# vituslcx/Shuffle-exchange

Measured on AMD Instinct MI355X. Metric: tokens/sec Llama-3-8B ZeRO-3 bf16 (training, whole job), higher is better.
Workload: dtype bf16; 1 GPU; llama8b-z3; model=llama3-8b, global_batch=16, seq_len=2048, micro_batch_per_gpu=8, grad_accum=2, parallelism=zero3-dp1, params=8030261248, activation_checkpointing=False, optimizer=AdamW(fp32 master, fused HIP), zero_knobs=tuned, sequence_parallel_size=1, expert_parallel_size=1

## Files before the change

csrc/kernels/flash_attn.hip:

```cpp
#include "sxe_common.h"
#include "sxe_mfma.h"
#include <torch/library.h>
#include <type_traits>

namespace sxe {
namespace fa {
using namespace mf;

constexpr int NW = 4;
constexpr int QW = 32;
constexpr int QB = NW * QW;
constexpr int KT = 64;

template <int D>
struct LaneOffs {
  int row[D / 16];
  int tr[D / 32][2];
  __device__ __forceinline__ void init(int lane) {
    const int r = lane & 31, h = lane >> 5;
#pragma unroll
    for (int t2 = 0; t2 < D / 16; ++t2) row[t2] = soff<D>(r, 2 * t2 + h);
    const int g = lane >> 4, i = lane & 15, q = i >> 2, p = i & 3, hh = g >> 1;
#pragma unroll
    for (int dt = 0; dt < D / 32; ++dt) {
      const int ch = 4 * dt + 2 * (g & 1) + (p >> 1);
      tr[dt][0] = soff<D>(4 * hh + q, ch) + 8 * (p & 1);
      tr[dt][1] = soff<D>(4 * hh + q + 8, ch) + 8 * (p & 1);
    }
  }
};
__device__ __forceinline__ bf16x8 lds_row_at(const char* base, int off) {
  return *reinterpret_cast<const bf16x8*>(base + off);
}
__device__ __forceinline__ bf16x8 lds_tr_at(const char* base, const int (&o)[2]) {
  return tr_pair(lds_tr(base, o[0]), lds_tr(base, o[1]));
}

struct Strides {
  int64_t b, s, h;
};

template <int ROWS, int NWAVES, int D>
struct Stager {
  static constexpr int CH = D / 8;
  static constexpr int N = ROWS * CH / (NWAVES * 64);
  u32x4 r[N];
  __device__ __forceinline__ void load(const unsigned short* base, int64_t row_stride, int row0, int nrows_valid) {
#pragma unroll
    for (int i = 0; i < N; ++i) {
      const int c = threadIdx.x + i * NWAVES * 64;
      const int row = c / CH, ch = c % CH;
      if (row0 + row < nrows_valid)
        r[i] = *reinterpret_cast<const u32x4*>(base + (int64_t)(row0 + row) * row_stride + ch * 8);
      else
        r[i] = u32x4{0, 0, 0, 0};
    }
  }
  __device__ __forceinline__ void store(char* lds) {
#pragma unroll
    for (int i = 0; i < N; ++i) {
      const int c = threadIdx.x + i * NWAVES * 64;
      const int row = c / CH, ch = c % CH;
      const int f = (((row & 3) << 2) | ((row >> 2) & 3)) & (CH >= 16 ? 15 : CH - 1);
      *reinterpret_cast<u32x4*>(lds + (row * (2 * D) + 16 * (ch ^ f))) = r[i];
    }
  }
};

struct Sparse {
  const uint8_t* layout;
  int blk, nb;
};

__device__ __forceinline__ int build_tile_list(const Sparse sp, int head, int t_lo, int t_hi, int tile, int r_lo,
                                               int r_hi, bool fixed_is_query, int* list) {
  int* flags = list + 1024;
  for (int t = t_lo + (int)threadIdx.x; t < t_hi; t += blockDim.x) {
    const int a0 = r_lo / sp.blk, a1 = (r_hi - 1) / sp.blk;
    const int b0 = (t * tile) / sp.blk, b1 = (t * tile + tile - 1) / sp.blk;
    int act = 0;
    for (int a = a0; a <= a1 && !act; ++a)
      for (int bb = b0; bb <= b1; ++bb) {
        const int qb_ = fixed_is_query ? a : bb, kb_ = fixed_is_query ? bb : a;
        if (sp.layout[((int64_t)head * sp.nb + qb_) * sp.nb + kb_]) { act = 1; break; }
      }
    flags[t - t_lo] = act;
  }
  __syncthreads();
  if (threadIdx.x == 0) {
    int n = 0;
    for (int t = t_lo; t < t_hi; ++t)
      if (flags[t - t_lo]) list[n++] = t;
    list[-1] = n;
  }
  __syncthreads();
  return list[-1];
}

struct Band {
  const int* klo;
  const int* qhi;
};
__device__ __forceinline__ int band_klo(const Band& bd, int b, int S, int i) {
  return min(max(bd.klo[(int64_t)b * S + i], 0), i);
}
__device__ __forceinline__ int band_qhi(const Band& bd, int b, int S, int j) {
  return max(min(bd.qhi[(int64_t)b * S + j], S - 1), j);
}

struct Varlen {
  const int* table;
  int T, window;
};

__device__ __forceinline__ void map_block(int nblk, int BH, bool heavy_last_index, int& bh, int& blk) {
  const int idx = blockIdx.x;
  const int rank = idx / BH;
  bh = idx - rank * BH;
  blk = heavy_last_index ? (nblk - 1 - rank) : rank;
}

extern __shared__ __attribute__((aligned(16))) char smem[];
__device__ __forceinline__ unsigned lds_addr(const char* p) {
  return __builtin_amdgcn_readfirstlane((unsigned)(uintptr_t)(__attribute__((address_space(3))) char*)smem +
                                        (unsigned)(p - smem));
}
template <int ROWS, int D, int NWV = NW, bool CLAMP = false>
__device__ __forceinline__ void tile_glds(const unsigned short* base, int64_t row_stride, int row0, char* lds,
                                          int rmax = 0) {
  constexpr int CH = D / 8, RPK = 64 / CH;
  static_assert(ROWS % (RPK * NWV) == 0, "tile rows must split evenly over the waves");
  const int lane = threadIdx.x & 63, w = __builtin_amdgcn_readfirstlane(threadIdx.x >> 6);
#pragma unroll
  for (int i = 0; i < ROWS / RPK / NWV; ++i) {
    const int n = i * NWV + w;
    const int row = RPK * n + lane / CH;
    const int cpos = lane % CH;
    const int ch = cpos ^ ((((row & 3) << 2) | ((row >> 2) & 3)) & (CH >= 16 ? 15 : CH - 1));
    const int grow = CLAMP ? min(row0 + row, rmax) : row0 + row;
    glds16_m0(base + (int64_t)grow * row_stride + ch * 8, lds_addr(lds + n * 1024));
  }
}


template <bool MASK, int D, bool BAND = false>
__device__ __forceinline__ void fwd_tile(const LaneOffs<D>& lo, const char* kt, const char* vt, const bf16x8 (&qf)[D / 16],
                                         f32x16 (&oacc)[D / 32], float& m, float& l, float c, int kbase, int qpos,
                                         int r, int h, int lane, bool diag, bool tail, int kvlen, const uint8_t* lrow,
                                         int blk, bool band = false, int kl = 0) {
  const bool skip1 = MASK && diag && !tail && lrow == nullptr && !(BAND && band) && kbase + 32 > qpos + QW - 1;
  f32x16 s[2];
#pragma unroll
  for (int j = 0; j < 2; ++j) {
    s[j] = zero16();
    if (j == 1 && skip1) break;
#pragma unroll
    for (int t2 = 0; t2 < D / 16; ++t2) s[j] = mfma(lds_row_at(kt + 32 * j * 2 * D, lo.row[t2]), qf[t2], s[j]);
  }
  float mx = -INFINITY;
  int dd = kbase + 4 * h - qpos - r, dl = kbase + 4 * h - kvlen;
  if (MASK) asm volatile("" : "+v"(dd), "+v"(dl));
  int db = kbase + 4 * h - kl;
  if (BAND) asm volatile("" : "+v"(db));
#pragma unroll
  for (int j = 0; j < 2; ++j) {
    bool b0 = true, b1 = true;
    if (MASK && lrow) {
      b0 = lrow[(kbase + 32 * j) / blk] != 0;
      b1 = lrow[(kbase + 32 * j + 16) / blk] != 0;
    }
#pragma unroll
    for (int i = 0; i < 16; ++i) {
      float x = s[j][i];
      if (MASK) {
        if (diag && dd + 32 * j + acc_row(i, 0) > 0) x = -INFINITY;
        if (tail && dl + 32 * j + acc_row(i, 0) >= 0) x = -INFINITY;
        if (!(i < 8 ? b0 : b1)) x = -INFINITY;
        if (BAND && band && db + 32 * j + acc_row(i, 0) < 0) x = -INFINITY;
        s[j][i] = x;
      }
      mx = fmaxf(mx, x);
    }
  }
  mx = fmaxf(mx, xor32(mx)) * c;
  const bool grow = mx > m + 8.f;
  const float mnew = grow ? mx : m;
  const float mref = (mnew == -INFINITY) ? 0.f : mnew;
  const float alpha = fast_exp2(m - mref);
  float ps = 0.f;
#pragma unroll
  for (int j = 0; j < 2; ++j)
#pragma unroll
    for (int i = 0; i < 16; ++i) {
      const float p = fast_exp2(__builtin_fmaf(s[j][i], c, -mref));
      s[j][i] = p;
      ps += p;
    }
  l = l * alpha + ps;
  m = mnew;
  if (__any(grow)) {
#pragma unroll
    for (int dt = 0; dt < D / 32; ++dt)
#pragma unroll
      for (int i = 0; i < 16; ++i) oacc[dt][i] *= alpha;
  }
#pragma unroll
  for (int j = 0; j < 2; ++j) {
    if (j == 1 && skip1) break;
#pragma unroll
    for (int s2 = 0; s2 < 2; ++s2) {
      const bf16x8 pb = acc_to_b(s[j], s2);
#pragma unroll
      for (int dt = 0; dt < D / 32; ++dt)
        oacc[dt] = mfma(lds_tr_at(vt + (32 * j + 16 * s2) * 2 * D, lo.tr[dt]), pb, oacc[dt]);
    }
  }
}

template <int D, int NWF>
constexpr int fwd_min_waves() { return D >= 256 ? 1 : 8 / NWF; }

template <bool SPARSE, int NWF, int D, bool DMA, bool BAND, bool VARLEN = false>
__device__ __forceinline__ void fwd_body(
    const unsigned short* __restrict__ q, Strides qs, const unsigned short* __restrict__ k, Strides ks,
    const unsigned short* __restrict__ v, Strides vs, unsigned short* __restrict__ o, Strides os,
    float* __restrict__ lse, int B, int H, int Hk, int Sq, int Sk, float scale, int causal, Sparse sp, int kvlen,
    int qoff, Band bd, Varlen vl = Varlen{nullptr, 0, 0}) {
  constexpr int ROWB = 2 * D;
  constexpr int BUF = 2 * KT * ROWB;
  int* tlist = reinterpret_cast<int*>(smem + 4 * KT * ROWB) + 1;
  constexpr int QBF = NWF * QW;
  const int lane = threadIdx.x & 63, w = threadIdx.x >> 6, r = lane & 31, h = lane >> 5;
  const int nqb = Sq / QBF;
  int bh, qb;
  if constexpr (VARLEN) {
    const int e = blockIdx.x / H;
    const int* te = vl.table + 3 * (int64_t)e;
    const int start = min(max(te[0], 0), vl.T - 1);
    Sq = Sk = kvlen = min(max(te[1], 1), vl.T - start);
    qb = min(max(te[2], 0), (Sq - 1) / QBF);
    bh = blockIdx.x - e * H;
    q += start * qs.s;
    k += start * ks.s;
    v += start * vs.s;
    o += start * os.s;
  } else {
    map_block(nqb, B * H, causal != 0, bh, qb);
  }
  const int b = bh / H, head = bh - b * H;
  const int kh = head / (H / Hk);
  const int q0 = qb * QBF + w * QW;
  const int qpos = q0 + qoff;
  const unsigned short* qp = q + b * qs.b + head * qs.h;
  const unsigned short* kp = k + b * ks.b + kh * ks.h;
  const unsigned short* vp = v + b * vs.b + kh * vs.h;
  const float c = scale * LOG2E;

  bf16x8 qf[D / 16];
#pragma unroll
  for (int t = 0; t < D / 16; ++t)
    qf[t] = *reinterpret_cast<const bf16x8*>(qp + (int64_t)(VARLEN ? min(q0 + r, Sq - 1) : q0 + r) * qs.s + 16 * t +
                                             8 * h);

  f32x16 oacc[D / 32];
#pragma unroll
  for (int t = 0; t < D / 32; ++t) oacc[t] = zero16();
  float m = -INFINITY, l = 0.f;

  const int kend = causal ? min(Sk, (qb + 1) * QBF + qoff) : Sk;
  const int nkt = (max(kend, 0) + KT - 1) / KT;
  auto klo_at = [&](int i) {
    if constexpr (VARLEN) return max(i - vl.window + 1, 0);
    else return band_klo(bd, b, Sq, i);
  };
  const int tfirst = BAND ? klo_at(qb * QBF) / KT : 0;
  const int kl = BAND ? klo_at(q0 + r) : 0;
  const int kl_lo = BAND ? __builtin_amdgcn_readfirstlane(kl) : 0;
  const int kl_hi = BAND ? __builtin_amdgcn_readlane(kl, QW - 1) : 0;
  const int ntiles = SPARSE ? build_tile_list(sp, head, 0, nkt, KT, qb * QBF, qb * QBF + QBF, true, tlist)
                            : (BAND ? nkt - tfirst : nkt);
  auto tile_at = [&](int i) { return SPARSE ? tlist[i] : (BAND ? tfirst + i : i); };
  const uint8_t* lrow = SPARSE ? sp.layout + ((int64_t)head * sp.nb + (q0 + r) / sp.blk) * sp.nb : nullptr;
  Stager<KT, NWF, D> sk, sv;
  const int t0 = ntiles > 0 ? tile_at(0) : 0;
  if constexpr (DMA) {
    if (ntiles > 0) {
      tile_glds<KT, D, NWF, VARLEN>(kp, ks.s, t0 * KT, smem, Sk - 1);
      tile_glds<KT, D, NWF, VARLEN>(vp, vs.s, t0 * KT, smem + KT * ROWB, Sk - 1);
    }
    vm_wait_all();
  } else {
    sk.load(kp, ks.s, t0 * KT, Sk);
    sv.load(vp, vs.s, t0 * KT, Sk);
    sk.store(smem);
    sv.store(smem + KT * ROWB);
  }
  __syncthreads();
  LaneOffs<D> lo;
  lo.init(lane);
  auto step = [&](const int t, auto slot) {
    constexpr int CUR = decltype(slot)::value;
    const bool more = (t + 1) < ntiles;
    if (more) {
      if constexpr (DMA) {
        tile_glds<KT, D, NWF, VARLEN>(kp, ks.s, tile_at(t + 1) * KT, smem + (CUR ^ 1) * BUF, Sk - 1);
        tile_glds<KT, D, NWF, VARLEN>(vp, vs.s, tile_at(t + 1) * KT, smem + (CUR ^ 1) * BUF + KT * ROWB, Sk - 1);
      } else {
        sk.load(kp, ks.s, tile_at(t + 1) * KT, Sk);
        sv.load(vp, vs.s, tile_at(t + 1) * KT, Sk);
      }
    }
    const int kbase = tile_at(t) * KT;
    const bool active = (!causal || kbase <= qpos + QW - 1) && !(BAND && kbase + KT - 1 < kl_lo) &&
                        !(VARLEN && q0 >= Sq);
    if (active) {
      const char* kt = smem + CUR * BUF;
      const char* vt = kt + KT * ROWB;
      const bool diag = causal && (kbase + KT - 1 > qpos);
      const bool tail = kbase + KT > kvlen;
      const bool band = BAND && kbase < kl_hi;
      if (SPARSE || diag || tail || band)
        fwd_tile<true, D, BAND>(lo, kt, vt, qf, oacc, m, l, c, kbase, qpos, r, h, lane, diag, tail, kvlen, lrow,
                                SPARSE ? sp.blk : 1, band, kl);
      else
        fwd_tile<false, D>(lo, kt, vt, qf, oacc, m, l, c, kbase, qpos, r, h, lane, false, false, kvlen, nullptr, 1);
    }
    if constexpr (DMA) {
      vm_wait_all();
    } else if (more) {
      sk.store(smem + (CUR ^ 1) * BUF);
      sv.store(smem + (CUR ^ 1) * BUF + KT * ROWB);
    }
    __syncthreads();
  };
  for (int t = 0; t < ntiles; t += 2) {
    step(t, std::integral_constant<int, 0>{});
    if (t + 1 < ntiles) step(t + 1, std::integral_constant<int, 1>{});
  }
  const float lt = l + __shfl_xor(l, 32, 64);
  const float inv = lt > 0.f ? 1.f / lt : 0.f;
  unsigned short* op = o + b * os.b + head * os.h + (int64_t)(q0 + r) * os.s;
  if (VARLEN && q0 + r >= Sq) return;
#pragma unroll
  for (int dt = 0; dt < D / 32; ++dt)
#pragma unroll
    for (int rg = 0; rg < 4; ++rg) {
      u16x4 pk;
#pragma unroll
      for (int e = 0; e < 4; ++e) pk[e] = f32_to_bf16(oacc[dt][4 * rg + e] * inv);
      *reinterpret_cast<u16x4*>(op + 32 * dt + 8 * rg + 4 * h) = pk;
    }
  if (VARLEN) return;
  if (h == 0) lse[((int64_t)b * H + head) * Sq + q0 + r] = lt > 0.f ? (m + log2f(lt)) * LN2 : INFINITY;
}

template <bool SPARSE, int NWF, int D, bool DMA = (D >= 256)>
__global__ void __launch_bounds__(NWF * 64, (fwd_min_waves<D, NWF>())) fwd_kernel(
    const unsigned short* __restrict__ q, Strides qs, const unsigned short* __restrict__ k, Strides ks,
    const unsigned short* __restrict__ v, Strides vs, unsigned short* __restrict__ o, Strides os,
    float* __restrict__ lse, int B, int H, int Hk, int Sq, int Sk, float scale, int causal, Sparse sp, int kvlen,
    int qoff) {
  fwd_body<SPARSE, NWF, D, DMA, false>(q, qs, k, ks, v, vs, o, os, lse, B, H, Hk, Sq, Sk, scale, causal, sp, kvlen,
                                       qoff, Band{nullptr, nullptr});
}

template <int NWF, int D>
__global__ void __launch_bounds__(NWF * 64, (fwd_min_waves<D, NWF>())) fwd_band_kernel(
    const unsigned short* __restrict__ q, Strides qs, const unsigned short* __restrict__ k, Strides ks,
    const unsigned short* __restrict__ v, Strides vs, unsigned short* __restrict__ o, Strides os,
    float* __restrict__ lse, int B, int H, int Hk, int S, float scale, Band bd) {
  fwd_body<false, NWF, D, true, true>(q, qs, k, ks, v, vs, o, os, lse, B, H, Hk, S, S, scale, 1,
                                      Sparse{nullptr, 0, 0}, S, 0, bd);
}

template <int D>
__global__ void __launch_bounds__(NW * 64, (fwd_min_waves<D, NW>())) fwd_varlen_kernel(
    const unsigned short* __restrict__ q, Strides qs, const unsigned short* __restrict__ k, Strides ks,
    const unsigned short* __restrict__ v, Strides vs, unsigned short* __restrict__ o, Strides os, int H, int Hk,
    float scale, Varlen vl) {
  fwd_body<false, NW, D, true, true, true>(q, qs, k, ks, v, vs, o, os, nullptr, 1, H, Hk, 0, 0, scale, 1,
                                           Sparse{nullptr, 0, 0}, 0, 0, Band{nullptr, nullptr}, vl);
}

template <int D>
__global__ void __launch_bounds__(256) delta_kernel(const unsigned short* __restrict__ dout, Strides ds,
                                                    const unsigned short* __restrict__ o, Strides os,
                                                    const float* __restrict__ lse, float* __restrict__ ndelta,
                                                    float* __restrict__ lse2, int B, int H, int S) {
  constexpr int TPR = D / 8, RPB = 256 / TPR;
  const int64_t row = (int64_t)blockIdx.x * RPB + (threadIdx.x / TPR);
  const int part = threadIdx.x % TPR;
  if (row >= (int64_t)B * H * S) return;
  const int s = (int)(row % S);
  const int64_t bh = row / S;
  const int hh = (int)(bh % H), b = (int)(bh / H);
  float x[8], y[8];
  load8<DT::BF16>(dout + b * ds.b + hh * ds.h + (int64_t)s * ds.s + part * 8, x);
  load8<DT::BF16>(o + b * os.b + hh * os.h + (int64_t)s * os.s + part * 8, y);
  float acc = 0.f;
#pragma unroll
  for (int e = 0; e < 8; ++e) acc += x[e] * y[e];
#pragma unroll
  for (int off = TPR / 2; off > 0; off >>= 1) acc += __shfl_xor(acc, off, TPR);
  if (part == 0) {
    ndelta[row] = -acc;
    lse2[row] = lse[row] * LOG2E;
  }
}

template <int D>
constexpr int bwd_min_waves() { return D >= 256 ? 1 : 2; }

template <bool MASK, int D, bool BAND = false>
__device__ __forceinline__ void dq_tile(const LaneOffs<D>& lo, const char* kt, const char* vt, const bf16x8 (&qf)[D / 16],
                                        const bf16x8 (&df)[D / 16], f32x16 (&dqacc)[D / 32], float c, float lse2,
                                        float ndlt, int kbase, int qpos, int r, int h, int lane, bool diag, bool tail,
                                        int kvlen, const uint8_t* lay_row, int blk, bool band = false,
                                        int kl = 0) {
  int dd = kbase + 4 * h - qpos - r, dl = kbase + 4 * h - kvlen;
  if (MASK) asm volatile("" : "+v"(dd), "+v"(dl));
  int db = kbase + 4 * h - kl;
  if (BAND) asm volatile("" : "+v"(db));
  const bool skip1 = MASK && diag && !tail && lay_row == nullptr && !(BAND && band) &&
                     kbase + 32 > qpos + QW - 1;
#pragma unroll
  for (int j = 0; j < 2; ++j) {
    if (j == 1 && skip1) break;
    f32x16 s = zero16(), dp = zero16();
#pragma unroll
    for (int t2 = 0; t2 < D / 16; ++t2) {
      s = mfma(lds_row_at(kt + 32 * j * 2 * D, lo.row[t2]), qf[t2], s);
      dp = mfma(lds_row_at(vt + 32 * j * 2 * D, lo.row[t2]), df[t2], dp);
    }
    bool b0 = true, b1 = true;
    if (MASK && lay_row) {
      b0 = lay_row[(kbase + 32 * j) / blk] != 0;
      b1 = lay_row[(kbase + 32 * j + 16) / blk] != 0;
    }
#pragma unroll
    for (int i = 0; i < 16; ++i) {
      float p = fast_exp2(__builtin_fmaf(s[i], c, -lse2));
      if (MASK) {
        if (diag && dd + 32 * j + acc_row(i, 0) > 0) p = 0.f;
        if (tail && dl + 32 * j + acc_row(i, 0) >= 0) p = 0.f;
        if (!(i < 8 ? b0 : b1)) p = 0.f;
        if (BAND && band && db + 32 * j + acc_row(i, 0) < 0) p = 0.f;
      }
      s[i] = p * (dp[i] + ndlt);
    }
#pragma unroll
    for (int s2 = 0; s2 < 2; ++s2) {
      const bf16x8 db = acc_to_b(s, s2);
#pragma unroll
      for (int dt = 0; dt < D / 32; ++dt)
        dqacc[dt] = mfma(lds_tr_at(kt + (32 * j + 16 * s2) * 2 * D, lo.tr[dt]), db, dqacc[dt]);
    }
  }
}

template <bool SPARSE, int D, int NWF, bool BAND>
__device__ __forceinline__ void dq_body(
    const unsigned short* __restrict__ q, Strides qs, const unsigned short* __restrict__ k, Strides ks,
    const unsigned short* __restrict__ v, Strides vs, const unsigned short* __restrict__ dout, Strides dos,
    const float* __restrict__ lse, const float* __restrict__ ndelta, unsigned short* __restrict__ dq, Strides dqs,
    int B, int H, int Hk, int Sq, int Sk, float scale, int causal, Sparse sp, int kvlen, int qoff, Band bd) {
  constexpr int ROWB = 2 * D;
  constexpr int BUF = 2 * KT * ROWB;
  int* tlist = reinterpret_cast<int*>(smem + 4 * KT * ROWB) + 1;
  const int lane = threadIdx.x & 63, w = threadIdx.x >> 6, r = lane & 31, h = lane >> 5;
  constexpr int QBF = NWF * QW;
  const int nqb = Sq / QBF;
  int bh, qb;
  map_block(nqb, B * H, causal != 0, bh, qb);
  const int b = bh / H, head = bh - b * H;
  const int kh = head / (H / Hk);
  const int q0 = qb * QBF + w * QW;
  const int qpos = q0 + qoff;
  const unsigned short* qp = q + b * qs.b + head * qs.h;
  const unsigned short* dop = dout + b * dos.b + head * dos.h;
  const unsigned short* kp = k + b * ks.b + kh * ks.h;
  const unsigned short* vp = v + b * vs.b + kh * vs.h;
  const float c = scale * LOG2E;
  const int64_t lrow = ((int64_t)b * H + head) * Sq + q0 + r;
  const int kend = causal ? min(Sk, (qb + 1) * QBF + qoff) : Sk;
  const int nkt = (max(kend, 0) + KT - 1) / KT;
  const int tfirst = BAND ? band_klo(bd, b, Sq, qb * QBF) / KT : 0;
  const int kl = BAND ? band_klo(bd, b, Sq, q0 + r) : 0;
  const int kl_lo = BAND ? __builtin_amdgcn_readfirstlane(kl) : 0;
  const int kl_hi = BAND ? __builtin_amdgcn_readlane(kl, QW - 1) : 0;
  const int ntiles = SPARSE ? build_tile_list(sp, head, 0, nkt, KT, qb * QBF, qb * QBF + QBF, true, tlist)
                            : (BAND ? nkt - tfirst : nkt);
  auto tile_at = [&](int i) { return SPARSE ? tlist[i] : (BAND ? tfirst + i : i); };
  const uint8_t* lay_row = SPARSE ? sp.layout + ((int64_t)head * sp.nb + (q0 + r) / sp.blk) * sp.nb : nullptr;
  if (ntiles > 0) {
    tile_glds<KT, D, NWF>(kp, ks.s, tile_at(0) * KT, smem);
    tile_glds<KT, D, NWF>(vp, vs.s, tile_at(0) * KT, smem + KT * ROWB);
  }

  const float lse2 = lse[lrow] * LOG2E;
  bf16x8 qf[D / 16], df[D / 16];
#pragma unroll
  for (int t = 0; t < D / 16; ++t) {
    qf[t] = *reinterpret_cast<const bf16x8*>(qp + (int64_t)(q0 + r) * qs.s + 16 * t + 8 * h);
    df[t] = *reinterpret_cast<const bf16x8*>(dop + (int64_t)(q0 + r) * dos.s + 16 * t + 8 * h);
  }
  const float ndlt = ndelta[lrow];
  f32x16 dqacc[D / 32];
#pragma unroll
  for (int t = 0; t < D / 32; ++t) dqacc[t] = zero16();
  vm_wait_all();
#pragma unroll
  for (int t = 0; t < D / 16; ++t) asm volatile("" ::"v"(qf[t]), "v"(df[t]));
  asm volatile("" ::"v"(lse2), "v"(ndlt));
  __syncthreads();
  LaneOffs<D> lo;
  lo.init(lane);
  auto step = [&](const int t, auto slot) {
    constexpr int CUR = decltype(slot)::value;
    if (t + 1 < ntiles) {
      tile_glds<KT, D, NWF>(kp, ks.s, tile_at(t + 1) * KT, smem + (CUR ^ 1) * BUF);
      tile_glds<KT, D, NWF>(vp, vs.s, tile_at(t + 1) * KT, smem + (CUR ^ 1) * BUF + KT * ROWB);
    }
    const int kbase = tile_at(t) * KT;
    const bool active = (!causal || kbase <= qpos + QW - 1) && !(BAND && kbase + KT - 1 < kl_lo);
    if (active) {
      const char* kt = smem + CUR * BUF;
      const char* vt = smem + CUR * BUF + KT * ROWB;
      const bool diag = causal && (kbase + KT - 1 > qpos);
      const bool tail = kbase + KT > kvlen;
      const bool band = BAND && kbase < kl_hi;
      if (SPARSE || diag || tail || band)
        dq_tile<true, D, BAND>(lo, kt, vt, qf, df, dqacc, c, lse2, ndlt, kbase, qpos, r, h, lane, diag, tail, kvlen,
                               lay_row, SPARSE ? sp.blk : 1, band, kl);
      else
        dq_tile<false, D>(lo, kt, vt, qf, df, dqacc, c, lse2, ndlt, kbase, qpos, r, h, lane, false, false, kvlen,
                          nullptr, 1);
    }
    vm_wait_all();
    __syncthreads();
  };
  for (int t = 0; t < ntiles; t += 2) {
    step(t, std::integral_constant<int, 0>{});
    if (t + 1 < ntiles) step(t + 1, std::integral_constant<int, 1>{});
  }
  unsigned short* op = dq + b * dqs.b + head * dqs.h + (int64_t)(q0 + r) * dqs.s;
#pragma unroll
  for (int dt = 0; dt < D / 32; ++dt)
#pragma unroll
    for (int rg = 0; rg < 4; ++rg) {
      u16x4 pk;
#pragma unroll
      for (int e = 0; e < 4; ++e) pk[e] = f32_to_bf16(dqacc[dt][4 * rg + e] * scale);
      *reinterpret_cast<u16x4*>(op + 32 * dt + 8 * rg + 4 * h) = pk;
    }
}

template <bool SPARSE, int D, int NWF = 4>
__global__ void __launch_bounds__(NWF * 64, (NWF == 8 ? 1 : bwd_min_waves<D>())) dq_kernel(
    const unsigned short* __restrict__ q, Strides qs, const unsigned short* __restrict__ k, Strides ks,
    const unsigned short* __restrict__ v, Strides vs, const unsigned short* __restrict__ dout, Strides dos,
    const float* __restrict__ lse, const float* __restrict__ ndelta, unsigned short* __restrict__ dq, Strides dqs,
    int B, int H, int Hk, int Sq, int Sk, float scale, int causal, Sparse sp, int kvlen, int qoff) {
  dq_body<SPARSE, D, NWF, false>(q, qs, k, ks, v, vs, dout, dos, lse, ndelta, dq, dqs, B, H, Hk, Sq, Sk, scale,
                                 causal, sp, kvlen, qoff, Band{nullptr, nullptr});
}

template <int D, int NWF = 4>
__global__ void __launch_bounds__(NWF * 64, (NWF == 8 ? 1 : bwd_min_waves<D>())) dq_band_kernel(
    const unsigned short* __restrict__ q, Strides qs, const unsigned short* __restrict__ k, Strides ks,
    const unsigned short* __restrict__ v, Strides vs, const unsigned short* __restrict__ dout, Strides dos,
    const float* __restrict__ lse, const float* __restrict__ ndelta, unsigned short* __restrict__ dq, Strides dqs,
    int B, int H, int Hk, int S, float scale, Band bd) {
  dq_body<false, D, NWF, true>(q, qs, k, ks, v, vs, dout, dos, lse, ndelta, dq, dqs, B, H, Hk, S, S, scale, 1,
                               Sparse{nullptr, 0, 0}, S, 0, bd);
}

constexpr int QT = 32;
template <int D, int KB = QB> struct KVL {
  static constexpr int TILE = QT * 2 * D;
  static constexpr int SLOT = 2 * TILE + 2 * QT * 4;
  static constexpr int VBLK = KB * 2 * D;
};

template <bool MASK, int D, int PART, bool BAND = false>
__device__ __forceinline__ void dkdv_tile(const LaneOffs<D>& lo, const char* slot, const char* vblk,
                                          const bf16x8 (&kf)[D / 16],
                                          f32x16 (&dka)[D / 32], f32x16 (&dva)[D / 32], float c, int qt0, int k0,
                                          int w, int r, int h, int lane, bool diag, const Sparse& sp, int hq0,
                                          int kbl, int qoff, bool band = false, int qh = 0) {
  const char* qt = slot;
  const char* dt_ = slot + KVL<D>::TILE;
  const float* l2 = reinterpret_cast<const float*>(slot + 2 * KVL<D>::TILE);
  const float* dl = l2 + QT;
  f32x16 s = zero16(), dp = zero16();
#pragma unroll
  for (int t2 = 0; t2 < D / 16; ++t2) {
    s = mfma(lds_row_at(qt, lo.row[t2]), kf[t2], s);
    if constexpr ((PART & 2) != 0)
      dp = mfma(lds_row_at(dt_, lo.row[t2]), lds_row_at(vblk + w * QW * 2 * D, lo.row[t2]), dp);
  }
  bool b0 = true, b1 = true;
  if (MASK && sp.layout) {
    b0 = sp.layout[((int64_t)hq0 * sp.nb + qt0 / sp.blk) * sp.nb + kbl] != 0;
    b1 = sp.layout[((int64_t)hq0 * sp.nb + (qt0 + 16) / sp.blk) * sp.nb + kbl] != 0;
  }
#pragma unroll
  for (int i = 0; i < 16; ++i) s[i] = fast_exp2(__builtin_fmaf(s[i], c, -l2[acc_row(i, h)]));
  if (MASK && diag) {
    int dd = k0 + r - 4 * h - qt0 - qoff;
    asm volatile("" : "+v"(dd));
#pragma unroll
    for (int i = 0; i < 16; ++i)
      if (dd > acc_row(i, 0)) s[i] = 0.f;
  }
  if (MASK && sp.layout) {
#pragma unroll
    for (int i = 0; i < 16; ++i)
      if (!(acc_row(i, h) < 16 ? b0 : b1)) s[i] = 0.f;
  }
  if (BAND && band) {
    int db = qh - qt0 - 4 * h;
    asm volatile("" : "+v"(db));
#pragma unroll
    for (int i = 0; i < 16; ++i)
      if (acc_row(i, 0) > db) s[i] = 0.f;
  }
#pragma unroll
  for (int i = 0; i < 16; ++i) dp[i] = s[i] * (dp[i] + dl[acc_row(i, h)]);
#pragma unroll
  for (int s2 = 0; s2 < 2; ++s2) {
    const bf16x8 pb = acc_to_b(s, s2);
    const bf16x8 db = acc_to_b(dp, s2);
#pragma unroll
    for (int t = 0; t < D / 32; ++t) {
      if constexpr ((PART & 1) != 0) dva[t] = mfma(lds_tr_at(dt_ + 16 * s2 * 2 * D, lo.tr[t]), pb, dva[t]);
      if constexpr ((PART & 2) != 0) dka[t] = mfma(lds_tr_at(qt + 16 * s2 * 2 * D, lo.tr[t]), db, dka[t]);
    }
  }
}

template <bool SPLIT, int D, int PART, int NWK, bool BAND>
__device__ __forceinline__ void dkdv_body(
    const unsigned short* __restrict__ q, Strides qs, const unsigned short* __restrict__ k, Strides ks,
    const unsigned short* __restrict__ v, Strides vs, const unsigned short* __restrict__ dout, Strides dos,
    const float* __restrict__ lse, const float* __restrict__ delta, unsigned short* __restrict__ dk, Strides dks,
    unsigned short* __restrict__ dv, Strides dvs, float* __restrict__ pk, float* __restrict__ pv, int B, int H,
    int Hk, int Sq, int Sk, float scale, int causal, Sparse sp, int qoff, int hpw, Band bd) {
  constexpr int KB = NWK * QW;
  using G_ = KVL<D, KB>;
  char* vblk = smem;
  char* ring = smem + G_::VBLK;
  int* tlist = reinterpret_cast<int*>(ring + 2 * G_::SLOT) + 1;
  const int lane = threadIdx.x & 63, w = __builtin_amdgcn_readfirstlane(threadIdx.x >> 6), r = lane & 31,
            h = lane >> 5;
  const int nkb = Sk / KB;
  int bh, kb;
  const int G = SPLIT ? hpw : H / Hk;
  const int HB = H / G;
  map_block(nkb, B * HB, false, bh, kb);
  const int b = bh / HB, hsel = bh - b * HB;
  const int hq0 = hsel * G;
  const int kh = hq0 / (H / Hk);
  const int k0 = kb * KB + w * QW;
  const unsigned short* kp = k + b * ks.b + kh * ks.h;
  const unsigned short* vp = v + b * vs.b + kh * vs.h;
  const float c = scale * LOG2E;
  const int qstart = causal ? min(Sq, max(0, kb * KB - qoff) / QT * QT) : 0;
  const int qend = BAND ? (band_qhi(bd, b, Sq, kb * KB + KB - 1) / QT + 1) * QT : Sq;
  const int qh = BAND ? band_qhi(bd, b, Sq, k0 + r) : 0;
  const int qh_lo = BAND ? __builtin_amdgcn_readfirstlane(qh) : 0;
  const int qh_hi = BAND ? __builtin_amdgcn_readlane(qh, QW - 1) : 0;
  const int ntq = (qend - qstart) / QT;
  const int total = sp.layout ? build_tile_list(sp, hq0, qstart / QT, Sq / QT, QT, kb * KB, kb * KB + KB, false, tlist)
                              : ntq * G;
  const int kbl = sp.layout ? (k0 + r) / sp.blk : 0;
  int is_h = hq0, is_q = qstart;
  int c_q = qstart;
  auto issue = [&](int it, char* slot) {
    const int hq = sp.layout ? hq0 : is_h;
    const int qt0 = sp.layout ? tlist[it] * QT : is_q;
    if (!sp.layout) {
      is_q += QT;
      if (is_q >= qend) {
        is_q = qstart;
        ++is_h;
      }
    }
    tile_glds<QT, D, NWK>(q + b * qs.b + hq * qs.h, qs.s, qt0, slot);
    tile_glds<QT, D, NWK>(dout + b * dos.b + hq * dos.h, dos.s, qt0, slot + G_::TILE);
    if (w == 0) {
      const int64_t lr = ((int64_t)b * H + hq) * Sq + qt0 + (lane & 31);
      glds4_m0(lane < 32 ? (const void*)(lse + lr) : (const void*)(delta + lr), lds_addr(slot + 2 * G_::TILE));
    }
  };
  if constexpr ((PART & 2) != 0) tile_glds<KB, D, NWK>(vp, vs.s, kb * KB, vblk);
  if (total > 0) issue(0, ring);
  bf16x8 kf[D / 16];
#pragma unroll
  for (int t = 0; t < D / 16; ++t)
    kf[t] = *reinterpret_cast<const bf16x8*>(kp + (int64_t)(k0 + r) * ks.s + 16 * t + 8 * h);
  f32x16 dka[D / 32], dva[D / 32];
#pragma unroll
  for (int t = 0; t < D / 32; ++t) {
    dka[t] = zero16();
    dva[t] = zero16();
  }
  vm_wait_all();
#pragma unroll
  for (int t = 0; t < D / 16; ++t) asm volatile("" ::"v"(kf[t]));
  __syncthreads();
  LaneOffs<D> lo;
  lo.init(lane);
  auto step = [&](const int it, auto slotc) {
    constexpr int CUR = decltype(slotc)::value;
    const int qt0 = sp.layout ? tlist[it] * QT : c_q;
    c_q = c_q + QT >= qend ? qstart : c_q + QT;
    const bool active = (!causal || (qt0 + QT - 1 + qoff >= k0)) && !(BAND && qt0 > qh_hi);
    const bool diag = causal && (qt0 + qoff < k0 + QW);
    const bool band = BAND && qt0 + QT - 1 > qh_lo;
    if (it + 1 < total) issue(it + 1, ring + (CUR ^ 1) * G_::SLOT);
    if (active)
      dkdv_tile<true, D, PART, BAND>(lo, ring + CUR * G_::SLOT, vblk, kf, dka, dva, c, qt0, k0, w, r, h, lane, diag,
                                     sp, hq0, kbl, qoff, band, qh);
    vm_wait_all();
    __syncthreads();
  };
  for (int it = 0; it < total; it += 2) {
    step(it, std::integral_constant<int, 0>{});
    if (it + 1 < total) step(it + 1, std::integral_constant<int, 1>{});
  }
  if (SPLIT && pk != nullptr) {
    float* kp32 = pk + (((int64_t)b * Sk + k0 + r) * HB + hsel) * D;
    float* vp32 = pv + (((int64_t)b * Sk + k0 + r) * HB + hsel) * D;
#pragma unroll
    for (int t = 0; t < D / 32; ++t)
#pragma unroll
      for (int rg = 0; rg < 4; ++rg) {
        f32x4 a, cc;
#pragma unroll
        for (int e = 0; e < 4; ++e) {
          a[e] = dka[t][4 * rg + e] * scale;
          cc[e] = dva[t][4 * rg + e];
        }
        if constexpr ((PART & 2) != 0) *reinterpret_cast<f32x4*>(kp32 + 32 * t + 8 * rg + 4 * h) = a;
        if constexpr ((PART & 1) != 0) *reinterpret_cast<f32x4*>(vp32 + 32 * t + 8 * rg + 4 * h) = cc;
      }
    return;
  }
  unsigned short* kop = dk + b * dks.b + kh * dks.h + (int64_t)(k0 + r) * dks.s;
  unsigned short* vop = dv + b * dvs.b + kh * dvs.h + (int64_t)(k0 + r) * dvs.s;
#pragma unroll
  for (int t = 0; t < D / 32; ++t)
#pragma unroll
    for (int rg = 0; rg < 4; ++rg) {
      u16x4 pk4, pv4;
#pragma unroll
      for (int e = 0; e < 4; ++e) {
        pk4[e] = f32_to_bf16(dka[t][4 * rg + e] * scale);
        pv4[e] = f32_to_bf16(dva[t][4 * rg + e]);
      }
      if constexpr ((PART & 2) != 0) *reinterpret_cast<u16x4*>(kop + 32 * t + 8 * rg + 4 * h) = pk4;
      if constexpr ((PART & 1) != 0) *reinterpret_cast<u16x4*>(vop + 32 * t + 8 * rg + 4 * h) = pv4;
    }
}

template <bool SPLIT, int D, int PART = 3, int NWK = 4>
__global__ void __launch_bounds__(NWK * 64, (NWK == 8 ? 1 : bwd_min_waves<D>())) dkdv_kernel(
    const unsigned short* __restrict__ q, Strides qs, const unsigned short* __restrict__ k, Strides ks,
    const unsigned short* __restrict__ v, Strides vs, const unsigned short* __restrict__ dout, Strides dos,
    const float* __restrict__ lse, const float* __restrict__ delta, unsigned short* __restrict__ dk, Strides dks,
    unsigned short* __restrict__ dv, Strides dvs, float* __restrict__ pk, float* __restrict__ pv, int B, int H,
    int Hk, int Sq, int Sk, float scale, int causal, Sparse sp, int qoff, int hpw) {
  dkdv_body<SPLIT, D, PART, NWK, false>(q, qs, k, ks, v, vs, dout, dos, lse, delta, dk, dks, dv, dvs, pk, pv, B, H,
                                        Hk, Sq, Sk, scale, causal, sp, qoff, hpw, Band{nullptr, nullptr});
}

template <bool SPLIT, int D, int PART = 3, int NWK = 4>
__global__ void __launch_bounds__(NWK * 64, (NWK == 8 ? 1 : bwd_min_waves<D>())) dkdv_band_kernel(
    const unsigned short* __restrict__ q, Strides qs, const unsigned short* __restrict__ k, Strides ks,
    const unsigned short* __restrict__ v, Strides vs, const unsigned short* __restrict__ dout, Strides dos,
    const float* __restrict__ lse, const float* __restrict__ delta, unsigned short* __restrict__ dk, Strides dks,
    unsigned short* __restrict__ dv, Strides dvs, float* __restrict__ pk, float* __restrict__ pv, int B, int H,
    int Hk, int S, float scale, int hpw, Band bd) {
  dkdv_body<SPLIT, D, PART, NWK, true>(q, qs, k, ks, v, vs, dout, dos, lse, delta, dk, dks, dv, dvs, pk, pv, B, H,
                                       Hk, S, S, scale, 1, Sparse{nullptr, 0, 0}, 0, hpw, bd);
}


template <int D>
__global__ void __launch_bounds__(256) dkdv_reduce_kernel(const float* __restrict__ pk, const float* __restrict__ pv,
                                                          unsigned short* __restrict__ dk, Strides dks,
                                                          unsigned short* __restrict__ dv, Strides dvs, int B, int S,
                                                          int H, int Hk) {
  const int G = H / Hk;
  const int64_t n8 = (int64_t)B * S * Hk * (D / 8);
  for (int64_t i = (int64_t)blockIdx.x * blockDim.x + threadIdx.x; i < n8; i += (int64_t)gridDim.x * blockDim.x) {
    const int c = (int)(i % (D / 8)) * 8;
    const int64_t rest = i / (D / 8);
    const int kh = (int)(rest % Hk);
    const int64_t bs = rest / Hk;
    const int b = (int)(bs / S), s_ = (int)(bs - (int64_t)b * S);
    float ak[8] = {0, 0, 0, 0, 0, 0, 0, 0}, av[8] = {0, 0, 0, 0, 0, 0, 0, 0};
    for (int g = 0; g < G; ++g) {
      const int64_t off = (bs * H + kh * G + g) * D + c;
      float x[8], y[8];
      load8<DT::F32>(pk + off, x);
      load8<DT::F32>(pv + off, y);
#pragma unroll
      for (int e = 0; e < 8; ++e) { ak[e] += x[e]; av[e] += y[e]; }
    }
    store8<DT::BF16>(dk + b * dks.b + (int64_t)s_ * dks.s + kh * dks.h + c, ak);
    store8<DT::BF16>(dv + b * dvs.b + (int64_t)s_ * dvs.s + kh * dvs.h + c, av);
  }
}

}

static fa::Strides strides_of(const at::Tensor& t) {
  return fa::Strides{t.stride(0), t.stride(1), t.stride(2)};
}
static unsigned short* u16(const at::Tensor& t) { return reinterpret_cast<unsigned short*>(t.data_ptr()); }

static void check_bf16_rows(std::initializer_list<const at::Tensor*> ts, const char* op) {
  for (const at::Tensor* t : ts) {
    bool ok = t->scalar_type() == at::kBFloat16 && t->stride(-1) == 1 &&
              (reinterpret_cast<uintptr_t>(t->data_ptr()) & 15) == 0;
    for (int64_t i = 0; i + 1 < t->dim(); ++i) ok = ok && t->stride(i) % 8 == 0;
    SXE_CHECK(ok, op, ": bf16 with unit stride on D and 16-byte aligned rows required");
  }
}

static void check_qkv(const at::Tensor& q, const at::Tensor& k, const at::Tensor& v) {
  SXE_CHECK(q.dim() == 4 && k.dim() == 4 && v.dim() == 4, "flash_attn: tensors must be [B, S, H, D]");
  check_bf16_rows({&q, &k, &v}, "flash_attn");
  const int64_t D = q.size(3);
  SXE_CHECK(D == 64 || D == 128 || D == 256, "flash_attn: head dim must be 64, 128 or 256");
  SXE_CHECK(k.size(3) == D && v.size(3) == D, "flash_attn: q/k/v head dims differ");
  SXE_CHECK(k.sizes() == v.sizes() && q.size(0) == k.size(0), "flash_attn: q/k/v shapes");
  SXE_CHECK(q.size(2) % k.size(2) == 0, "flash_attn: Hq must be a multiple of Hkv");
  SXE_CHECK(q.size(1) % fa::QB == 0 && k.size(1) % fa::QB == 0, "flash_attn: seq lengths must be multiples of 128");
}

static fa::Sparse sparse_of(const c10::optional<at::Tensor>& layout, int64_t block, const at::Tensor& q) {
  if (!layout.has_value() || !layout->defined()) return fa::Sparse{nullptr, 0, 0};
  const at::Tensor& L = *layout;
  const int S = q.size(1), H = q.size(2);
  SXE_CHECK(L.is_cuda() && L.scalar_type() == at::kByte && L.is_contiguous() && L.dim() == 3, "layout: uint8 [H, nb, nb]");
  SXE_CHECK(block >= 16 && block % 16 == 0 && S % block == 0, "layout block must be a multiple of 16 dividing seq_len");
  SXE_CHECK(L.size(0) == H && L.size(1) == S / block && L.size(2) == S / block, "layout shape must be [H, S/block, S/block]");
  SXE_CHECK(S / fa::KT <= 1024, "sparse attention: seq_len <= 65536");
  return fa::Sparse{L.data_ptr<uint8_t>(), (int)block, (int)(S / block)};
}

static fa::Band band_of(const at::Tensor& klo, const at::Tensor& qhi, const at::Tensor& q, const at::Tensor& k) {
  SXE_CHECK(q.dim() == 4 && k.dim() == 4 && q.size(1) == k.size(1), "flash_attn band: needs Sq == Sk");
  for (const at::Tensor* t : {&klo, &qhi})
    SXE_CHECK(t->is_cuda() && t->device() == q.device() && t->scalar_type() == at::kInt && t->is_contiguous() &&
                  t->dim() == 2 && t->size(0) == q.size(0) && t->size(1) == q.size(1),
              "flash_attn band: klo / qhi must be contiguous int32 [B, S] on the device of q");
  return fa::Band{klo.data_ptr<int>(), qhi.data_ptr<int>()};
}

constexpr size_t kListBytes = (1 + 2048) * sizeof(int) + 16;

static int env_int(const char* name, int dflt) {
  const char* e = std::getenv(name);
  return (e != nullptr && *e != 0) ? std::atoi(e) : dflt;
}

template <int D> constexpr size_t kRingBytes = 4 * fa::KT * 2 * D;

template <auto Kernel> using kern_t = std::integral_constant<decltype(Kernel), Kernel>;
template <int N> using int_t = std::integral_constant<int, N>;

template <auto Kernel, typename... Args>
static void launch(int grid, int waves, size_t lds, Args... args) {
  allow_max_dynamic_lds<Kernel>();
  hipLaunchKernelGGL(Kernel, dim3(grid), dim3(waves * 64), lds, cur_stream(), args...);
  SXE_LAUNCH_CHECK();
}

struct Mask {
  bool causal;
  int kvlen, qoff;
  fa::Sparse sp;
  fa::Band bd;
};
constexpr fa::Sparse kNoSparse{nullptr, 0, 0};
constexpr fa::Band kNoBand{nullptr, nullptr};

static Mask mask_of(const at::Tensor& q, const at::Tensor& k, bool causal, fa::Sparse sp, int64_t kv_len,
                    int64_t causal_offset, fa::Band bd) {
  const int Sq = q.size(1), Sk = k.size(1);
  const int kvlen = kv_len < 0 ? Sk : (int)kv_len;
  SXE_CHECK(kvlen >= 1 && kvlen <= Sk, "flash_attn: kv_len must be in [1, Sk]");
  const int qoff = causal_offset == INT64_MIN ? Sk - Sq : (int)causal_offset;
  SXE_CHECK(!sp.layout || (Sq == Sk && qoff == 0), "block-sparse attention needs Sq == Sk");
  SXE_CHECK(!bd.klo || (causal && Sq == Sk && qoff == 0 && kvlen == Sk && !sp.layout),
            "flash_attn band: needs causal, Sq == Sk, causal offset 0, no kv_len and no sparse layout");
  return Mask{causal, kvlen, qoff, sp, bd};
}

template <int D>
static std::vector<at::Tensor> fwd_impl_d(const at::Tensor& q, const at::Tensor& k, const at::Tensor& v, double scale,
                                          const Mask& m) {
  static_assert(kRingBytes<D> + kListBytes <= kMaxDynamicLds, "forward LDS exceeds the opt-in limit");
  const int B = q.size(0), Sq = q.size(1), H = q.size(2), Sk = k.size(1), Hk = k.size(2);
  auto o = at::empty({B, Sq, H, D}, q.options());
  auto lse = at::empty({B, H, Sq}, q.options().dtype(at::kFloat));
  const size_t lds = kRingBytes<D> + (m.sp.layout ? kListBytes : 0);
  const int grid = (Sq / fa::QB) * B * H;
  auto run = [&](auto nwf, auto dma) {
    constexpr int NWF = decltype(nwf)::value;
    constexpr bool DMA = decltype(dma)::value;
    auto go = [&](auto kern, auto... tail) {
      launch<decltype(kern)::value>(NWF == 8 ? grid / 2 : grid, NWF, lds, u16(q), strides_of(q), u16(k), strides_of(k),
                                    u16(v), strides_of(v), u16(o), strides_of(o), lse.data_ptr<float>(), B, H, Hk, Sq,
                                    tail...);
    };
    auto dense = [&](auto kern) { go(kern, Sk, (float)scale, m.causal ? 1 : 0, m.sp, m.kvlen, m.qoff); };
    if (m.bd.klo != nullptr) go(kern_t<fa::fwd_band_kernel<NWF, D>>{}, (float)scale, m.bd);
    else if (m.sp.layout != nullptr) dense(kern_t<fa::fwd_kernel<true, NWF, D, DMA>>{});
    else dense(kern_t<fa::fwd_kernel<false, NWF, D, DMA>>{});
  };
  if constexpr (D < 256) {
    const bool wide = Sq % 256 == 0 && env_int("SXE_FA_FWD_WAVES", 8) != 4;
    const bool dma = m.bd.klo != nullptr || env_int("SXE_FA_FWD_DMA", 1) != 0;
    if (wide) dma ? run(int_t<8>{}, std::true_type{}) : run(int_t<8>{}, std::false_type{});
    else dma ? run(int_t<4>{}, std::true_type{}) : run(int_t<4>{}, std::false_type{});
  } else {
    run(int_t<4>{}, std::true_type{});
  }
  return {o, lse};
}

static std::vector<at::Tensor> fwd_impl(at::Tensor q, at::Tensor k, at::Tensor v, bool causal, double scale,
                                        fa::Sparse sp, int64_t kv_len = -1, int64_t causal_offset = INT64_MIN,
                                        fa::Band bd = kNoBand) {
  check_qkv(q, k, v);
  const Mask m = mask_of(q, k, causal, sp, kv_len, causal_offset, bd);
  c10::DeviceGuard guard(q.device());
  std::vector<at::Tensor> out;
  dispatch_head_dim(q.size(3), "flash_attn", [&](auto d) { out = fwd_impl_d<decltype(d)::value>(q, k, v, scale, m); });
  return out;
}

template <int D>
static void bwd_impl_d(const at::Tensor& dout, const at::Tensor& q, const at::Tensor& k, const at::Tensor& v,
                       const at::Tensor& o, const at::Tensor& lse, const at::Tensor& dq, const at::Tensor& dk,
                       const at::Tensor& dv, double scale, const Mask& m) {
  using G_ = fa::KVL<D>;
  constexpr int KB8 = D == 128 ? 256 : fa::QB;
  static_assert(kRingBytes<D> + kListBytes <= kMaxDynamicLds, "dQ LDS exceeds the opt-in limit");
  static_assert(fa::KVL<D, KB8>::VBLK + 2 * G_::SLOT + kListBytes <= kMaxDynamicLds,
                "dK/dV LDS exceeds the opt-in limit");
  const bool causal = m.causal;
  const fa::Sparse sp = m.sp;
  const int B = q.size(0), Sq = q.size(1), H = q.size(2), Sk = k.size(1), Hk = k.size(2);
  auto ndelta = at::empty({B, H, Sq}, q.options().dtype(at::kFloat));
  auto lse2 = at::empty({B, H, Sq}, q.options().dtype(at::kFloat));
  const int64_t rows = (int64_t)B * H * Sq;
  constexpr int RPB = 256 / (D / 8);
  hipLaunchKernelGGL(fa::delta_kernel<D>, dim3((rows + RPB - 1) / RPB), dim3(256), 0, cur_stream(), u16(dout),
                     strides_of(dout), u16(o), strides_of(o), lse.data_ptr<float>(), ndelta.data_ptr<float>(),
                     lse2.data_ptr<float>(), B, H, Sq);
  SXE_LAUNCH_CHECK();
  const size_t lds_dq = kRingBytes<D> + (sp.layout ? kListBytes : 0);
  auto run_dq = [&](auto nwf) {
    constexpr int NWF = decltype(nwf)::value;
    auto go = [&](auto kern, auto... tail) {
      launch<decltype(kern)::value>((Sq / (NWF * fa::QW)) * B * H, NWF, lds_dq, u16(q), strides_of(q), u16(k),
                                    strides_of(k), u16(v), strides_of(v), u16(dout), strides_of(dout),
                                    lse.data_ptr<float>(), ndelta.data_ptr<float>(), u16(dq), strides_of(dq), B, H, Hk,
                                    Sq, tail...);
    };
    auto dense = [&](auto kern) { go(kern, Sk, (float)scale, causal ? 1 : 0, sp, m.kvlen, m.qoff); };
    if (m.bd.klo != nullptr) go(kern_t<fa::dq_band_kernel<D, NWF>>{}, (float)scale, m.bd);
    else if (sp.layout != nullptr) dense(kern_t<fa::dq_kernel<true, D, NWF>>{});
    else dense(kern_t<fa::dq_kernel<false, D, NWF>>{});
  };
  const int dqw = env_int("SXE_FA_DQ_WAVES", 0);
  const bool dq8 = D < 256 && Sq % 256 == 0 && (dqw == 8 || (dqw == 0 && Sq >= 8192));
  if constexpr (D < 256) {
    dq8 ? run_dq(int_t<8>{}) : run_dq(int_t<4>{});
  } else {
    run_dq(int_t<4>{});
  }
  int hpw = sp.layout != nullptr ? 1 : env_int("SXE_FA_DKDV_HPW", 0);
  if (hpw == 0) {
    int64_t cap = (int64_t)B * H * (Sk / fa::QB) / (4 * kNumCUs);
    if (Sk >= 8192 && cap > 2) cap = 2;
    for (int d = H / Hk; d >= 1; --d)
      if ((H / Hk) % d == 0 && d <= cap) {
        hpw = d;
        break;
      }
  }
  if (hpw < 1 || (H / Hk) % hpw != 0) hpw = 1;
  const bool split = sp.layout != nullptr || (causal && H / Hk > hpw);
  const bool partials = split && H / hpw > Hk;
  const int np = H / hpw;
  const bool one_sweep = D >= 256 && env_int("SXE_FA_DKDV_ONE_SWEEP", 1) != 0;
  const int kvw = env_int("SXE_FA_DKDV_WAVES", 0);
  const bool kv8 = D == 128 && Sk % 256 == 0 && (kvw == 8 || (kvw == 0 && Sk >= 8192));
  const size_t lds_kv = (kv8 ? fa::KVL<D, 256>::VBLK : G_::VBLK) + 2 * G_::SLOT + (sp.layout ? kListBytes : 0);
  at::Tensor pk, pv;
  if (partials) {
    pk = at::empty({B, Sk, np, D}, q.options().dtype(at::kFloat));
    pv = at::empty({B, Sk, np, D}, q.options().dtype(at::kFloat));
  }
  auto run = [&](auto splitc, auto part, auto nwk, int heads) {
    constexpr bool SP = decltype(splitc)::value;
    constexpr int PART = decltype(part)::value, NWK = decltype(nwk)::value;
    auto go = [&](auto kern, auto... tail) {
      launch<decltype(kern)::value>((Sk / (NWK * fa::QW)) * B * heads, NWK, lds_kv, u16(q), strides_of(q), u16(k),
                                    strides_of(k), u16(v), strides_of(v), u16(dout), strides_of(dout),
                                    lse2.data_ptr<float>(), ndelta.data_ptr<float>(), u16(dk), strides_of(dk), u16(dv),
                                    strides_of(dv), partials ? pk.data_ptr<float>() : nullptr,
                                    partials ? pv.data_ptr<float>() : nullptr, B, H, Hk, Sq, tail...);
    };
    if (m.bd.klo != nullptr) go(kern_t<fa::dkdv_band_kernel<SP, D, PART, NWK>>{}, (float)scale, hpw, m.bd);
    else go(kern_t<fa::dkdv_kernel<SP, D, PART, NWK>>{}, Sk, (float)scale, causal ? 1 : 0, sp, m.qoff, hpw);
  };
  auto run_dkdv = [&](auto splitc, int heads) {
    if constexpr (D >= 256) {
      if (!one_sweep) {
        run(splitc, int_t<1>{}, int_t<4>{}, heads);
        run(splitc, int_t<2>{}, int_t<4>{}, heads);
        return;
      }
    }
    if constexpr (D == 128) {
      if (kv8) {
        run(splitc, int_t<3>{}, int_t<8>{}, heads);
        return;
      }
    }
    run(splitc, int_t<3>{}, int_t<4>{}, heads);
  };
  if (split) {
    run_dkdv(std::true_type{}, np);
    if (partials) {
      const int64_t n8 = (int64_t)B * Sk * Hk * (D / 8);
      hipLaunchKernelGGL(fa::dkdv_reduce_kernel<D>, dim3(stream_grid(n8, 256)), dim3(256), 0, cur_stream(),
                         pk.data_ptr<float>(), pv.data_ptr<float>(), u16(dk), strides_of(dk), u16(dv), strides_of(dv),
                         B, Sk, np, Hk);
      SXE_LAUNCH_CHECK();
    }
  } else {
    run_dkdv(std::false_type{}, Hk);
  }
}

static void bwd_impl(at::Tensor dout, at::Tensor q, at::Tensor k, at::Tensor v, at::Tensor o, at::Tensor lse,
                     at::Tensor dq, at::Tensor dk, at::Tensor dv, bool causal, double scale, fa::Sparse sp,
                     int64_t kv_len = -1, int64_t causal_offset = INT64_MIN,
                     fa::Band bd = kNoBand) {
  check_qkv(q, k, v);
  check_qkv(dq, dk, dv);
  const Mask m = mask_of(q, k, causal, sp, kv_len, causal_offset, bd);
  SXE_CHECK(dout.sizes() == q.sizes() && o.sizes() == q.sizes() && dout.stride(3) == 1 && o.stride(3) == 1,
            "flash_attn_bwd: dout/o shapes");
  SXE_CHECK(dq.sizes() == q.sizes() && dk.sizes() == k.sizes() && dv.sizes() == v.sizes(), "flash_attn_bwd: grad shapes");
  SXE_CHECK(lse.is_contiguous() && lse.size(2) == q.size(1), "flash_attn_bwd: lse [B, H, Sq]");
  c10::DeviceGuard guard(q.device());
  dispatch_head_dim(q.size(3), "flash_attn_bwd", [&](auto d) {
    bwd_impl_d<decltype(d)::value>(dout, q, k, v, o, lse, dq, dk, dv, scale, m);
  });
}

static int64_t offset_arg(int64_t causal_offset) { return causal_offset == -(int64_t(1) << 40) ? INT64_MIN : causal_offset; }

std::vector<at::Tensor> flash_attn_fwd(at::Tensor q, at::Tensor k, at::Tensor v, bool causal, double scale,
                                       int64_t kv_len, int64_t causal_offset) {
  return fwd_impl(q, k, v, causal, scale, kNoSparse, kv_len, offset_arg(causal_offset));
}

void flash_attn_bwd(at::Tensor dout, at::Tensor q, at::Tensor k, at::Tensor v, at::Tensor o, at::Tensor lse,
                    at::Tensor dq, at::Tensor dk, at::Tensor dv, bool causal, double scale, int64_t kv_len,
                    int64_t causal_offset) {
  bwd_impl(dout, q, k, v, o, lse, dq, dk, dv, causal, scale, kNoSparse, kv_len, offset_arg(causal_offset));
}

std::vector<at::Tensor> flash_attn_fwd_sparse(at::Tensor q, at::Tensor k, at::Tensor v, at::Tensor layout,
                                              int64_t block, bool causal, double scale) {
  return fwd_impl(q, k, v, causal, scale, sparse_of(layout, block, q));
}

void flash_attn_bwd_sparse(at::Tensor dout, at::Tensor q, at::Tensor k, at::Tensor v, at::Tensor o, at::Tensor lse,
                           at::Tensor dq, at::Tensor dk, at::Tensor dv, at::Tensor layout, int64_t block, bool causal,
                           double scale) {
  bwd_impl(dout, q, k, v, o, lse, dq, dk, dv, causal, scale, sparse_of(layout, block, q));
}

std::vector<at::Tensor> flash_attn_fwd_band(at::Tensor q, at::Tensor k, at::Tensor v, at::Tensor klo, at::Tensor qhi,
                                            double scale) {
  return fwd_impl(q, k, v, true, scale, kNoSparse, -1, INT64_MIN, band_of(klo, qhi, q, k));
}

void flash_attn_bwd_band(at::Tensor dout, at::Tensor q, at::Tensor k, at::Tensor v, at::Tensor o, at::Tensor lse,
                         at::Tensor dq, at::Tensor dk, at::Tensor dv, at::Tensor klo, at::Tensor qhi, double scale) {
  bwd_impl(dout, q, k, v, o, lse, dq, dk, dv, true, scale, kNoSparse, -1, INT64_MIN, band_of(klo, qhi, q, k));
}

template <int D>
static void fwd_varlen_d(const at::Tensor& q, const at::Tensor& k, const at::Tensor& v, const at::Tensor& o,
                         const at::Tensor& table, double scale, int window) {
  static_assert(kRingBytes<D> <= kMaxDynamicLds, "varlen LDS exceeds the opt-in limit");
  auto st = [](const at::Tensor& t) { return fa::Strides{0, t.stride(0), t.stride(1)}; };
  const int H = q.size(1), N = table.size(0);
  launch<fa::fwd_varlen_kernel<D>>(N * H, fa::NW, kRingBytes<D>, u16(q), st(q), u16(k), st(k), u16(v), st(v), u16(o),
                                   st(o), H, (int)k.size(1), (float)scale,
                                   fa::Varlen{table.data_ptr<int>(), (int)q.size(0), window});
}

at::Tensor flash_attn_fwd_varlen(at::Tensor q, at::Tensor k, at::Tensor v, at::Tensor table, double scale,
                                 int64_t window, c10::optional<at::Tensor> out) {
  SXE_CHECK(q.dim() == 3 && k.dim() == 3 && v.dim() == 3, "flash_attn varlen: tensors must be [T, H, D]");
  SXE_CHECK(q.is_cuda() && k.device() == q.device() && v.device() == q.device(), "flash_attn varlen: q/k/v on one GPU");
  const int64_t T = q.size(0), H = q.size(1), D = q.size(2);
  SXE_CHECK(D == 64 || D == 128 || D == 256, "flash_attn varlen: head dim must be 64, 128 or 256");
  SXE_CHECK(k.size(2) == D && v.size(2) == D, "flash_attn varlen: q/k/v head dims differ");
  SXE_CHECK(k.sizes() == v.sizes() && k.size(0) == T, "flash_attn varlen: q/k/v shapes");
  SXE_CHECK(k.size(1) >= 1 && H % k.size(1) == 0, "flash_attn varlen: Hq must be a multiple of Hkv");
  SXE_CHECK(T < (int64_t(1) << 31) / 3, "flash_attn varlen: too many tokens");
  SXE_CHECK(window >= 0, "flash_attn varlen: window must be >= 0 (0 = none)");
  SXE_CHECK(table.is_cuda() && table.device() == q.device() && table.scalar_type() == at::kInt && table.dim() == 2 &&
                table.size(1) == 3 && table.is_contiguous(),
            "flash_attn varlen: table must be contiguous int32 [N, 3] on the device of q");
  SXE_CHECK(table.size(0) * H < (int64_t(1) << 31), "flash_attn varlen: table too long");
  at::Tensor o = out.has_value() && out->defined() ? *out : at::empty({T, H, D}, q.options());
  SXE_CHECK(o.dim() == 3 && o.sizes() == q.sizes() && o.scalar_type() == at::kBFloat16 && o.device() == q.device(),
            "flash_attn varlen: out must be bf16 [T, Hq, D] on the device of q");
  check_bf16_rows({&q, &k, &v, &o}, "flash_attn varlen");
  if (T == 0 || table.size(0) == 0) return o;
  c10::DeviceGuard guard(q.device());
  const int w = window == 0 ? (1 << 30) : (int)std::min<int64_t>(window, 1 << 30);
  dispatch_head_dim(D, "flash_attn varlen", [&](auto d) { fwd_varlen_d<decltype(d)::value>(q, k, v, o, table, scale, w); });
  return o;
}

}

TORCH_LIBRARY_FRAGMENT(sxe, m) {
  m.def("flash_attn_fwd(Tensor q, Tensor k, Tensor v, bool causal, float scale, int kv_len=-1, "
        "int causal_offset=-1099511627776) -> Tensor[]");
  m.def("flash_attn_bwd(Tensor dout, Tensor q, Tensor k, Tensor v, Tensor o, Tensor lse, Tensor(a!) dq, Tensor(b!) dk, "
        "Tensor(c!) dv, bool causal, float scale, int kv_len=-1, int causal_offset=-1099511627776) -> ()");
  m.def("flash_attn_fwd_sparse(Tensor q, Tensor k, Tensor v, Tensor layout, int block, bool causal, float scale) -> Tensor[]");
  m.def("flash_attn_bwd_sparse(Tensor dout, Tensor q, Tensor k, Tensor v, Tensor o, Tensor lse, Tensor(a!) dq, "
        "Tensor(b!) dk, Tensor(c!) dv, Tensor layout, int block, bool causal, float scale) -> ()");
  m.def("flash_attn_fwd_band(Tensor q, Tensor k, Tensor v, Tensor klo, Tensor qhi, float scale) -> Tensor[]");
  m.def("flash_attn_bwd_band(Tensor dout, Tensor q, Tensor k, Tensor v, Tensor o, Tensor lse, Tensor(a!) dq, "
        "Tensor(b!) dk, Tensor(c!) dv, Tensor klo, Tensor qhi, float scale) -> ()");
  m.def("flash_attn_fwd_varlen(Tensor q, Tensor k, Tensor v, Tensor table, float scale, int window=0, "
        "Tensor(a!)? out=None) -> Tensor");
}
TORCH_LIBRARY_IMPL(sxe, CUDA, m) {
  m.impl("flash_attn_fwd", &sxe::flash_attn_fwd);
  m.impl("flash_attn_bwd", &sxe::flash_attn_bwd);
  m.impl("flash_attn_fwd_sparse", &sxe::flash_attn_fwd_sparse);
  m.impl("flash_attn_bwd_sparse", &sxe::flash_attn_bwd_sparse);
  m.impl("flash_attn_fwd_band", &sxe::flash_attn_fwd_band);
  m.impl("flash_attn_bwd_band", &sxe::flash_attn_bwd_band);
  m.impl("flash_attn_fwd_varlen", &sxe::flash_attn_fwd_varlen);
}
```

csrc/kernels/transpose.hip:

```cpp
#include "sxe_common.h"
#include <torch/library.h>

namespace sxe {

constexpr int TT = 64;
constexpr int TLD = TT + 2;

__global__ void __launch_bounds__(256) transpose16_kernel(const unsigned short* __restrict__ x,
                                                          unsigned short* __restrict__ y, int64_t R, int64_t C) {
  __shared__ unsigned short tile[TT * TLD];
  const int64_t tiles_c = C / TT;
  const int64_t tr = blockIdx.x / tiles_c, tc = blockIdx.x - tr * tiles_c;
  const int t = threadIdx.x;
  const int r = t >> 2, c0 = (t & 3) * 16;
  const unsigned short* src = x + (tr * TT + r) * C + tc * TT + c0;
  const u16x8 a = *reinterpret_cast<const u16x8*>(src);
  const u16x8 b = *reinterpret_cast<const u16x8*>(src + 8);
#pragma unroll
  for (int j = 0; j < 8; ++j) {
    tile[r * TLD + c0 + j] = a[j];
    tile[r * TLD + c0 + 8 + j] = b[j];
  }
  __syncthreads();
  const int oc = t >> 2, r0 = (t & 3) * 16;
  u16x8 o0, o1;
#pragma unroll
  for (int j = 0; j < 8; ++j) {
    o0[j] = tile[(r0 + j) * TLD + oc];
    o1[j] = tile[(r0 + 8 + j) * TLD + oc];
  }
  unsigned short* dst = y + (tc * TT + oc) * R + tr * TT + r0;
  *reinterpret_cast<u16x8*>(dst) = o0;
  *reinterpret_cast<u16x8*>(dst + 8) = o1;
}

at::Tensor transpose16(at::Tensor x) {
  SXE_CHECK_CUDA(x);
  SXE_CHECK(x.dim() == 2 && x.is_contiguous(), "transpose16: contiguous 2-D input");
  SXE_CHECK(x.element_size() == 2, "transpose16: 16-bit dtype");
  const int64_t R = x.size(0), C = x.size(1);
  SXE_CHECK(R % TT == 0 && C % TT == 0, "transpose16: dims must be multiples of 64");
  c10::DeviceGuard guard(x.device());
  auto y = at::empty({C, R}, x.options());
  const int64_t tiles = (R / TT) * (C / TT);
  if (tiles == 0) return y;
  SXE_CHECK(tiles < (1ll << 31), "transpose16: too many tiles");
  hipLaunchKernelGGL(transpose16_kernel, dim3((unsigned)tiles), dim3(256), 0, cur_stream(),
                     reinterpret_cast<const unsigned short*>(x.data_ptr()),
                     reinterpret_cast<unsigned short*>(y.data_ptr()), R, C);
  SXE_LAUNCH_CHECK();
  return y;
}

}

TORCH_LIBRARY_FRAGMENT(sxe, m) { m.def("transpose16(Tensor x) -> Tensor"); }
TORCH_LIBRARY_IMPL(sxe, CUDA, m) { m.impl("transpose16", &sxe::transpose16); }
```

shuffle_exchange_amd/ops/attention.py:

```python
import math
import os

import torch
import torch.nn.functional as F

from . import native
from ..utils.logging import warning_once


def band_bounds(S, B, device, position_ids=None, doc_ids=None, window=None):
    if position_ids is None and doc_ids is None and window is None:
        return None
    idx = torch.arange(S, device=device, dtype=torch.int32).expand(B, S)
    klo = torch.zeros(B, S, dtype=torch.int32, device=device)
    qhi = torch.full((B, S), S - 1, dtype=torch.int32, device=device)
    start = None
    if position_ids is not None:
        start = (position_ids.to(device).reshape(-1, S) == 0).expand(B, S)
    if doc_ids is not None:
        d = doc_ids.to(device).reshape(-1, S).expand(B, S)
        chg = torch.ones(B, S, dtype=torch.bool, device=device)
        chg[:, 1:] = d[:, 1:] != d[:, :-1]
        start = chg if start is None else (start | chg)
    if start is not None:
        zero = torch.zeros_like(idx)
        klo = torch.cummax(torch.where(start, idx, zero), dim=1).values.to(torch.int32)
        nxt = torch.full((B, S + 1), S, dtype=torch.int32, device=device)
        nxt[:, :S] = torch.where(start, idx, torch.full_like(idx, S))
        nxt = torch.cummin(nxt.flip(1), dim=1).values.flip(1)
        qhi = (nxt[:, 1:] - 1).to(torch.int32)
    if window is not None:
        W = int(window)
        if W < 1:
            raise ValueError(f"window must be >= 1, got {window}")
        klo = torch.maximum(klo, (idx - (W - 1)).clamp_min(0))
        qhi = torch.minimum(qhi, (idx + (W - 1)).clamp_max(S - 1))
    return klo.contiguous(), qhi.contiguous()


def band_mask(bounds, S):
    klo = bounds[0]
    i = torch.arange(S, device=klo.device)
    lo = torch.minimum(klo.long().clamp_min(0), i)
    return (i[None, None, :] >= lo[:, :, None]) & (i[None, None, :] <= i[None, :, None])


def _check_band(q, k, causal, bounds):
    if not causal or q.shape[1] != k.shape[1]:
        raise ValueError("attention bounds need causal=True and equal query / key lengths")
    klo, qhi = bounds
    if tuple(klo.shape) != (q.shape[0], q.shape[1]) or tuple(qhi.shape) != tuple(klo.shape):
        raise ValueError(f"attention bounds must be [B, S] = {(q.shape[0], q.shape[1])}, got {tuple(klo.shape)}")


def _sdpa(q, k, v, causal, scale, mask=None):
    if mask is not None:
        qt, kt, vt = q.transpose(1, 2), k.transpose(1, 2), v.transpose(1, 2)
        if qt.shape[1] != kt.shape[1]:
            rep = qt.shape[1] // kt.shape[1]
            kt, vt = kt.repeat_interleave(rep, dim=1), vt.repeat_interleave(rep, dim=1)
        o = F.scaled_dot_product_attention(qt, kt, vt, attn_mask=mask[:, None], scale=scale)
        return o.transpose(1, 2)
    qt, kt, vt = q.transpose(1, 2), k.transpose(1, 2), v.transpose(1, 2)
    gqa = qt.shape[1] != kt.shape[1]
    if gqa and not q.is_cuda:
        rep = qt.shape[1] // kt.shape[1]
        kt = kt.repeat_interleave(rep, dim=1)
        vt = vt.repeat_interleave(rep, dim=1)
        gqa = False
    o = F.scaled_dot_product_attention(qt, kt, vt, is_causal=causal, scale=scale, enable_gqa=gqa)
    return o.transpose(1, 2)


TILE = 128
HEAD_DIMS = (64, 128, 256)


def _native_dim(D):
    for d in HEAD_DIMS:
        if d >= D:
            return d
    return None


def _aligned(t):
    ok = t.stride(-1) == 1 and t.stride(0) % 8 == 0 and t.stride(1) % 8 == 0 and t.stride(2) % 8 == 0
    if torch.compiler.is_compiling():
        return ok
    return ok and (t.storage_offset() * t.element_size()) % 16 == 0


def hip_supported(q, k, v):
    if os.environ.get("SXE_ATTN_BACKEND") == "sdpa":
        return False
    return (q.is_cuda and q.dtype == torch.bfloat16 and q.shape[-1] in HEAD_DIMS and q.shape[1] % TILE == 0
            and k.shape[1] % TILE == 0 and k.shape[-1] == q.shape[-1] and v.shape[-1] == q.shape[-1]
            and q.shape[2] % k.shape[2] == 0 and _aligned(q) and _aligned(k) and _aligned(v))


def hip_paddable(q, k, v):
    if os.environ.get("SXE_ATTN_BACKEND") == "sdpa":
        return False
    return (q.is_cuda and q.dtype in (torch.bfloat16, torch.float16, torch.float32)
            and _native_dim(q.shape[-1]) is not None and q.shape[-1] % 8 == 0 and k.shape[-1] == q.shape[-1]
            and v.shape[-1] == q.shape[-1] and q.shape[2] % k.shape[2] == 0)


def _pad(t, S_pad, D_pad):
    B, S, H, D = t.shape
    if S == S_pad and D == D_pad and t.dtype == torch.bfloat16 and _aligned(t):
        return t
    out = torch.zeros(B, S_pad, H, D_pad, dtype=torch.bfloat16, device=t.device)
    out[:, :S, :, :D].copy_(t)
    return out


def _flash_fwd(q, k, v, causal, scale, klo, qhi, *kv_args):
    if klo is not None:
        return torch.ops.sxe.flash_attn_fwd_band(q, k, v, klo, qhi, float(scale))
    return torch.ops.sxe.flash_attn_fwd(q, k, v, bool(causal), float(scale), *kv_args)


def _flash_bwd(do, q, k, v, o, lse, dq, dk, dv, causal, scale, klo, qhi, *kv_args):
    if klo is not None:
        torch.ops.sxe.flash_attn_bwd_band(do, q, k, v, o, lse, dq, dk, dv, klo, qhi, float(scale))
    else:
        torch.ops.sxe.flash_attn_bwd(do, q, k, v, o, lse, dq, dk, dv, bool(causal), float(scale), *kv_args)


def _pad_bounds(bounds, S_pad):
    klo, qhi = bounds
    B, S = klo.shape
    if S == S_pad:
        return klo, qhi
    kp = torch.full((B, S_pad), S, dtype=torch.int32, device=klo.device)
    qp = torch.full((B, S_pad), S_pad - 1, dtype=torch.int32, device=klo.device)
    kp[:, :S] = klo
    qp[:, :S] = qhi.clamp_max(S - 1)
    return kp, qp


def _padded_kv_args(Sq, Sk, klo):
    return (Sk, Sk - Sq) if klo is None else ()


def _padded_fwd(q, k, v, causal, scale, klo=None, qhi=None):
    Sq, Sk, D = q.shape[1], k.shape[1], q.shape[-1]
    Dp = _native_dim(D)
    Sqp, Skp = -(-Sq // TILE) * TILE, -(-Sk // TILE) * TILE
    qp, kp, vp = _pad(q, Sqp, Dp), _pad(k, Skp, Dp), _pad(v, Skp, Dp)
    if klo is not None:
        klo, qhi = _pad_bounds((klo, qhi), Sqp)
    o, lse = _flash_fwd(qp, kp, vp, causal, scale, klo, qhi, *_padded_kv_args(Sq, Sk, klo))
    return qp, kp, vp, o, lse, klo, qhi


class _FlashAttnPadded(torch.autograd.Function):

    @staticmethod
    def forward(ctx, q, k, v, causal, scale, klo, qhi):
        Sq, Sk, D = q.shape[1], k.shape[1], q.shape[-1]
        qp, kp, vp, o, lse, klo, qhi = _padded_fwd(q, k, v, causal, scale, klo, qhi)
        ctx.save_for_backward(qp, kp, vp, o, lse, klo, qhi)
        ctx.meta = (causal, scale, Sq, Sk, D, q.dtype)
        return o[:, :Sq, :, :D].to(q.dtype)

    @staticmethod
    def backward(ctx, do):
        qp, kp, vp, o, lse, klo, qhi = ctx.saved_tensors
        causal, scale, Sq, Sk, D, dtype = ctx.meta
        dop = _pad(do, qp.shape[1], qp.shape[-1])
        dq, dk, dv = torch.empty_like(qp), torch.empty_like(kp), torch.empty_like(vp)
        _flash_bwd(dop, qp, kp, vp, o, lse, dq, dk, dv, causal, scale, klo, qhi, *_padded_kv_args(Sq, Sk, klo))
        sq = (slice(None), slice(0, Sq), slice(None), slice(0, D))
        sk = (slice(None), slice(0, Sk), slice(None), slice(0, D))
        return dq[sq].to(dtype), dk[sk].to(dtype), dv[sk].to(dtype), None, None, None, None


class _FlashAttn(torch.autograd.Function):
    @staticmethod
    def forward(ctx, q, k, v, causal, scale, klo, qhi):
        o, lse = _flash_fwd(q, k, v, causal, scale, klo, qhi)
        ctx.save_for_backward(q, k, v, o, lse, klo, qhi)
        ctx.causal, ctx.scale = causal, scale
        return o

    @staticmethod
    def backward(ctx, do):
        q, k, v, o, lse, klo, qhi = ctx.saved_tensors
        dq, dk, dv = torch.empty_like(q), torch.empty_like(k), torch.empty_like(v)
        _flash_bwd(do.contiguous(), q, k, v, o, lse, dq, dk, dv, ctx.causal, ctx.scale, klo, qhi)
        return dq, dk, dv, None, None, None, None


def attention(q, k, v, causal=True, softmax_scale=None, bounds=None):
    scale = softmax_scale if softmax_scale is not None else 1.0 / math.sqrt(q.shape[-1])
    klo, qhi = None, None
    if bounds is not None:
        _check_band(q, k, causal, bounds)
        klo, qhi = bounds
    if q.is_cuda:
        native.require_hip()
        if hip_supported(q, k, v):
            return _FlashAttn.apply(q, k, v, causal, scale, klo, qhi)
        if hip_paddable(q, k, v):
            return _FlashAttnPadded.apply(q, k, v, causal, scale, klo, qhi)
        warning_once(f"sxe attention: HIP flash kernel does not cover dtype={q.dtype} D={q.shape[-1]} "
                     f"S={q.shape[1]}; using SDPA")
    return _sdpa(q, k, v, causal, scale, band_mask(bounds, q.shape[1]) if bounds is not None else None)


class _FlashAttnQKVRope(torch.autograd.Function):
    @staticmethod
    def forward(ctx, qkv, cos, sin, nq, nkv, causal, scale, pos, klo, qhi):
        B, S = qkv.shape[0], qkv.shape[1]
        if cos is not None:
            torch.ops.sxe.rope_(qkv[:, :, :nq + nkv], cos, sin, pos, S, 0, False)
        q, k, v = qkv[:, :, :nq], qkv[:, :, nq:nq + nkv], qkv[:, :, nq + nkv:]
        o, lse = _flash_fwd(q, k, v, causal, scale, klo, qhi)
        ctx.save_for_backward(qkv, o, lse, cos, sin, pos, klo, qhi)
        ctx.meta = (nq, nkv, causal, scale)
        return o

    @staticmethod
    def backward(ctx, do):
        qkv, o, lse, cos, sin, pos, klo, qhi = ctx.saved_tensors
        nq, nkv, causal, scale = ctx.meta
        dqkv = torch.empty_like(qkv)
        q, k, v = qkv[:, :, :nq], qkv[:, :, nq:nq + nkv], qkv[:, :, nq + nkv:]
        dq, dk, dv = dqkv[:, :, :nq], dqkv[:, :, nq:nq + nkv], dqkv[:, :, nq + nkv:]
        _flash_bwd(do.contiguous(), q, k, v, o, lse, dq, dk, dv, causal, scale, klo, qhi)
        if cos is not None:
            torch.ops.sxe.rope_(dqkv[:, :, :nq + nkv], cos, sin, pos, qkv.shape[1], 0, True)
        return dqkv, None, None, None, None, None, None, None, None, None


def attention_qkv_rope(qkv, nq, nkv, rope=None, position_ids=None, causal=True, softmax_scale=None, bounds=None):
    D = qkv.shape[-1]
    scale = softmax_scale if softmax_scale is not None else 1.0 / math.sqrt(D)
    q, k, v = qkv[:, :, :nq], qkv[:, :, nq:nq + nkv], qkv[:, :, nq + nkv:]
    if qkv.is_cuda:
        native.require_hip()
        if hip_supported(q, k, v):
            pos = position_ids.reshape(-1).contiguous().long() if position_ids is not None else None
            cos = rope.cos if rope is not None else None
            sin = rope.sin if rope is not None else None
            klo, qhi = None, None
            if bounds is not None:
                _check_band(q, k, causal, bounds)
                klo, qhi = bounds
            return _FlashAttnQKVRope.apply(qkv, cos, sin, nq, nkv, causal, scale, pos, klo, qhi)
    if rope is not None:
        from .rope import apply_rope_qkv_
        qkv = apply_rope_qkv_(qkv, rope, nq + nkv, position_ids)
    q, k, v = qkv[:, :, :nq], qkv[:, :, nq:nq + nkv], qkv[:, :, nq + nkv:]
    return attention(q, k, v, causal, scale, bounds)


QKV_TN = os.environ.get("SXE_QKV_TN", "1") == "1"


class _QKVProjAttn(torch.autograd.Function):

    @staticmethod
    def forward(ctx, x, w, cos, sin, nq, nkv, causal, scale, pos, klo, qhi):
        B, S, H = x.shape
        x2 = x.reshape(-1, H)
        qkv = F.linear(x2, w).view(B, S, nq + 2 * nkv, -1)
        if cos is not None:
            torch.ops.sxe.rope_(qkv[:, :, :nq + nkv], cos, sin, pos, S, 0, False)
        q, k, v = qkv[:, :, :nq], qkv[:, :, nq:nq + nkv], qkv[:, :, nq + nkv:]
        o, lse = _flash_fwd(q, k, v, causal, scale, klo, qhi)
        xT = torch.ops.sxe.transpose16(x2) if ctx.needs_input_grad[1] else None
        ctx.save_for_backward(xT, qkv, o, lse, cos, sin, pos, w, klo, qhi)
        ctx.meta = (nq, nkv, causal, scale, x.shape)
        return o

    @staticmethod
    def backward(ctx, do):
        xT, qkv, o, lse, cos, sin, pos, w, klo, qhi = ctx.saved_tensors
        nq, nkv, causal, scale, x_shape = ctx.meta
        dqkv = torch.empty_like(qkv)
        q, k, v = qkv[:, :, :nq], qkv[:, :, nq:nq + nkv], qkv[:, :, nq + nkv:]
        dq, dk, dv = dqkv[:, :, :nq], dqkv[:, :, nq:nq + nkv], dqkv[:, :, nq + nkv:]
        _flash_bwd(do.contiguous(), q, k, v, o, lse, dq, dk, dv, causal, scale, klo, qhi)
        del q, k, v, o, lse, qkv
        if cos is not None:
            torch.ops.sxe.rope_(dqkv[:, :, :nq + nkv], cos, sin, pos, dqkv.shape[1], 0, True)
        d2 = dqkv.view(-1, w.shape[0])
        from .linear import data_grad
        from .mlp import weight_grad_tn
        dx = data_grad(d2, w).view(x_shape) if ctx.needs_input_grad[0] else None
        dw = None
        if ctx.needs_input_grad[1]:
            dw = weight_grad_tn(w, torch.ops.sxe.transpose16(d2), xT, fp32_out=True)
        return dx, dw, None, None, None, None, None, None, None, None, None


def qkv_proj_attention(x, qkv_proj, nq, nkv, rope=None, position_ids=None, causal=True, softmax_scale=None,
                       bounds=None):
    B, S, H = x.shape
    w = getattr(qkv_proj, "weight", None)
    from .mlp import _plain
    N = (nq + 2 * nkv)
    if (QKV_TN and x.is_cuda and x.dtype == torch.bfloat16 and torch.is_grad_enabled() and _plain(qkv_proj)
            and (w.requires_grad or x.requires_grad) and (B * S) % 64 == 0 and H % 64 == 0 and w.shape[1] == H
            and w.shape[0] % (64 * N) == 0 and native.use_hip(x)):
        D = w.shape[0] // N
        if D in HEAD_DIMS and S % TILE == 0 and nq % nkv == 0 and os.environ.get("SXE_ATTN_BACKEND") != "sdpa":
            scale = softmax_scale if softmax_scale is not None else 1.0 / math.sqrt(D)
            pos = position_ids.reshape(-1).contiguous().long() if position_ids is not None else None
            cos = rope.cos if rope is not None else None
            sin = rope.sin if rope is not None else None
            klo, qhi = None, None
            if bounds is not None:
                klo, qhi = bounds
                if not causal or tuple(klo.shape) != (B, S) or tuple(qhi.shape) != (B, S):
                    raise ValueError("attention bounds need causal=True and [B, S] tensors")
            return _QKVProjAttn.apply(x, w, cos, sin, nq, nkv, causal, scale, pos, klo, qhi)
    qkv = qkv_proj(x).view(B, S, N, -1)
    return attention_qkv_rope(qkv, nq, nkv, rope, position_ids, causal, softmax_scale, bounds)


def attention_with_lse(q, k, v, causal=True, softmax_scale=None):
    scale = softmax_scale if softmax_scale is not None else 1.0 / math.sqrt(q.shape[-1])
    if q.is_cuda and hip_supported(q, k, v):
        return torch.ops.sxe.flash_attn_fwd(q, k, v, bool(causal), float(scale))
    if q.is_cuda and hip_paddable(q, k, v):
        Sq, D = q.shape[1], q.shape[-1]
        o, lse = _padded_fwd(q, k, v, causal, scale)[3:5]
        return o[:, :Sq, :, :D].to(q.dtype), lse[:, :, :Sq].contiguous()
    return reference_attention(q, k, v, causal, scale, return_lse=True)


def varlen_hip_supported(q, k, v, out=None):
    if os.environ.get("SXE_ATTN_BACKEND") == "sdpa" or not native.use_hip(q):
        return False
    ts = (q, k, v) if out is None else (q, k, v, out)
    return (q.dim() == 3 and q.shape[-1] in HEAD_DIMS and k.shape[-1] == q.shape[-1] and v.shape[-1] == q.shape[-1]
            and k.shape[1] > 0 and q.shape[1] % k.shape[1] == 0
            and all(t.dtype == torch.bfloat16 and t.stride(2) == 1 and t.stride(0) % 8 == 0 and t.stride(1) % 8 == 0
                    and (t.storage_offset() * t.element_size()) % 16 == 0 for t in ts))


def varlen_attention(q, k, v, table, scale=None, window=None, out=None):
    scale = scale if scale is not None else 1.0 / math.sqrt(q.shape[-1])
    if window is not None and int(window) < 1:
        raise ValueError(f"window must be >= 1, got {window}")
    if q.is_cuda:
        native.require_hip()
        if varlen_hip_supported(q, k, v, out):
            return torch.ops.sxe.flash_attn_fwd_varlen(q, k, v, table, float(scale), int(window or 0), out)
        warning_once(f"sxe varlen attention: HIP kernel does not cover dtype={q.dtype} D={q.shape[-1]} "
                     f"strides={q.stride()}; using the per-sequence reference")
    if out is None:
        out = torch.zeros_like(q)
    for s, n in dict.fromkeys((int(r[0]), int(r[1])) for r in table.tolist()):
        sl = slice(s, s + n)
        bounds = band_bounds(n, 1, q.device, window=window) if window is not None and window < n else None
        out[sl] = reference_attention(q[sl][None], k[sl][None], v[sl][None], True, scale, bounds=bounds)[0]
    return out


def reference_attention(q, k, v, causal=True, scale=None, return_lse=False, bounds=None):
    scale = scale if scale is not None else 1.0 / math.sqrt(q.shape[-1])
    qt, kt, vt = q.transpose(1, 2).float(), k.transpose(1, 2).float(), v.transpose(1, 2).float()
    if kt.shape[1] != qt.shape[1]:
        rep = qt.shape[1] // kt.shape[1]
        kt, vt = kt.repeat_interleave(rep, 1), vt.repeat_interleave(rep, 1)
    s = torch.matmul(qt, kt.transpose(-1, -2)) * scale
    if causal:
        S, T = s.shape[-2], s.shape[-1]
        mask = torch.ones(S, T, dtype=torch.bool, device=s.device).tril(T - S)
        s = s.masked_fill(~mask, float("-inf"))
    if bounds is not None:
        _check_band(q, k, causal, bounds)
        s = s.masked_fill(~band_mask(bounds, s.shape[-1])[:, None], float("-inf"))
    lse = torch.logsumexp(s, dim=-1)
    o = torch.matmul(torch.softmax(s, dim=-1), vt).transpose(1, 2).to(q.dtype)
    return (o, lse) if return_lse else o
```

shuffle_exchange_amd/ops/fake_kernels.py:

```python
import torch

from . import native

native.require_hip()
_reg = torch.library.register_fake


def _rows(x):
    return x.numel() // x.shape[-1]


@_reg("sxe::norm_fwd")
def _norm_fwd(x, residual, weight, bias, eps, layernorm):
    r = _rows(x)
    f = x.new_empty((r,), dtype=torch.float32)
    mean = x.new_empty((r,) if layernorm else (0,), dtype=torch.float32)
    h = torch.empty_like(x) if residual is not None else x.new_empty((0,))
    return [torch.empty_like(x), f, mean, h]


@_reg("sxe::norm_bwd")
def _norm_bwd(dy, x, rstd, mean, weight, dres, layernorm):
    H = x.shape[-1]
    return [torch.empty_like(x), x.new_empty((H,), dtype=torch.float32),
            x.new_empty((H,) if layernorm else (0,), dtype=torch.float32)]


@_reg("sxe::rope_")
def _rope(x, cos, sin, pos, seq_len, pos_offset, inverse):
    return None


@_reg("sxe::gated_act_fwd")
def _gated_fwd(gu, act):
    return gu.new_empty(gu.shape[:-1] + (gu.shape[-1] // 2,))


@_reg("sxe::gated_act_bwd")
def _gated_bwd(dout, gu, act):
    return torch.empty_like(gu)


@_reg("sxe::gated_act_fwd_dual")
def _gated_fwd_dual(gu, act, variant=0):
    I = gu.shape[-1] // 2
    T = gu.numel() // gu.shape[-1]
    return gu.new_empty(gu.shape[:-1] + (I,)), gu.new_empty((I, T))


@_reg("sxe::gated_act_bwd_dual")
def _gated_bwd_dual(dout, gu, act, variant=0):
    T = gu.numel() // gu.shape[-1]
    return torch.empty_like(gu), gu.new_empty((gu.shape[-1], T))


@_reg("sxe::bias_act_fwd")
def _bias_act_fwd(x, bias, act):
    return torch.empty_like(x)


@_reg("sxe::bias_act_bwd")
def _bias_act_bwd(dy, x, bias, act):
    return torch.empty_like(x)


@_reg("sxe::flash_attn_fwd")
def _fa_fwd(q, k, v, causal, scale, kv_len=-1, causal_offset=-(1 << 40)):
    B, Sq, H, D = q.shape
    return [q.new_empty((B, Sq, H, v.shape[-1])), q.new_empty((B, H, Sq), dtype=torch.float32)]


@_reg("sxe::flash_attn_bwd")
def _fa_bwd(dout, q, k, v, o, lse, dq, dk, dv, causal, scale, kv_len=-1, causal_offset=-(1 << 40)):
    return None


@_reg("sxe::flash_attn_fwd_band")
def _fa_fwd_band(q, k, v, klo, qhi, scale):
    B, Sq, H, D = q.shape
    return [q.new_empty((B, Sq, H, v.shape[-1])), q.new_empty((B, H, Sq), dtype=torch.float32)]


@_reg("sxe::flash_attn_bwd_band")
def _fa_bwd_band(dout, q, k, v, o, lse, dq, dk, dv, klo, qhi, scale):
    return None


@_reg("sxe::flash_attn_fwd_varlen")
def _fa_fwd_varlen(q, k, v, table, scale, window=0, out=None):
    return torch.empty_like(q, memory_format=torch.contiguous_format)


@_reg("sxe::xent_fwd")
def _xent_fwd(logits, target, ignore_index, inplace_grad, scale, grad_scale):
    r = logits.shape[0]
    return logits.new_empty((r,), dtype=torch.float32), logits.new_empty((r,), dtype=torch.float32)


@_reg("sxe::xent_bwd")
def _xent_bwd(logits, target, lse, dloss, ignore_index, inplace):
    return torch.empty_like(logits)


@_reg("sxe::xent_grad_dual")
def _xent_grad_dual(logits, target, lse, ignore_index, scale_a, scale_b):
    return logits.new_empty((logits.shape[1], logits.shape[0]))


@_reg("sxe::acc2_bf16_")
def _acc2(dst, a, b, accumulate):
    return None


@_reg("sxe::transpose16")
def _transpose16(x):
    return x.new_empty((x.shape[1], x.shape[0]))


@_reg("sxe::wgrad_gemm_")
def _wgrad(a, b, c, alpha, accumulate):
    return None


@_reg("sxe::gather_rows")
def _gather_rows(src, idx, offset=0, add=None):
    return src.new_empty((idx.numel(),) + tuple(src.shape[1:]))


@_reg("sxe::fake_quant")
def _fake_quant(x, groups, mode, bits, range=None):
    return torch.empty_like(x)


@_reg("sxe::scatter_rows_")
def _scatter_rows(dst, idx, src):
    return None
```

Before: 26030 tokens/s.

## Fuse inverse RoPE and transposed dQKV write into flash-attention backward epilogue

Adds epilogue variants of the dQ and dK/dV backward kernels that apply scaling and inverse RoPE directly to the fp32 accumulators. They can also write a transposed copy of dQKV through an LDS tile for the weight-gradient GEMM. This removes the separate rope_ in-place pass and the standalone transpose16 kernel over the dqkv buffer, cutting extra memory round-trips. The cost is more LDS syncs and extra stores inside the attention kernels. The fused path is taken only for non-sparse, non-8-wave, square-sequence cases.

```diff
diff --git a/csrc/kernels/flash_attn.hip b/csrc/kernels/flash_attn.hip
--- a/csrc/kernels/flash_attn.hip
+++ b/csrc/kernels/flash_attn.hip
@@ -411,6 +411,79 @@
 template <int D>
 constexpr int bwd_min_waves() { return D >= 256 ? 1 : 2; }
 
+struct RopeBwd {
+  const float* cos;
+  const float* sin;
+  const int64_t* pos;
+  int max_pos;
+  int rot_heads_q, rot_heads_k;
+};
+struct DualT {
+  unsigned short* q;
+  unsigned short* k;
+  unsigned short* v;
+  int64_t ld;
+};
+struct BwdEpi {
+  RopeBwd rope;
+  DualT dt;
+};
+
+template <int D>
+__device__ __forceinline__ void rope_inv_acc(f32x16 (&x)[D / 32], const RopeBwd& rp, int64_t tok, int s, int h) {
+  constexpr int HALF = D / 2, HT = D / 64;
+  int64_t p = rp.pos ? rp.pos[tok] : (int64_t)s;
+  p = p < 0 ? 0 : (p >= rp.max_pos ? (int64_t)rp.max_pos - 1 : p);
+  const float* cs = rp.cos + p * HALF + 4 * h;
+  const float* sn = rp.sin + p * HALF + 4 * h;
+#pragma unroll
+  for (int dt = 0; dt < HT; ++dt)
+#pragma unroll
+    for (int rg = 0; rg < 4; ++rg) {
+      const f32x4 c4 = *reinterpret_cast<const f32x4*>(cs + 32 * dt + 8 * rg);
+      const f32x4 s4 = *reinterpret_cast<const f32x4*>(sn + 32 * dt + 8 * rg);
+#pragma unroll
+      for (int e = 0; e < 4; ++e) {
+        const float a = x[dt][4 * rg + e], b = x[dt + HT][4 * rg + e];
+        x[dt][4 * rg + e] = a * c4[e] + b * s4[e];
+        x[dt + HT][4 * rg + e] = b * c4[e] - a * s4[e];
+      }
+    }
+}
+
+constexpr int TSTR = 288;
+template <int D> constexpr int kTileBytes = D * TSTR;
+
+template <int D>
+__device__ __forceinline__ void tile_put(char* tile, const u16x4 (&pk)[D / 32][4], int w, int r, int h) {
+  const bool odd = (r & 1) != 0;
+#pragma unroll
+  for (int dt = 0; dt < D / 32; ++dt)
+#pragma unroll
+    for (int rg = 0; rg < 4; ++rg) {
+      const unsigned lo = (unsigned)pk[dt][rg][0] | ((unsigned)pk[dt][rg][1] << 16);
+      const unsigned hi = (unsigned)pk[dt][rg][2] | ((unsigned)pk[dt][rg][3] << 16);
+      const unsigned got = (unsigned)__shfl_xor((int)(odd ? lo : hi), 1);
+      const unsigned keep = odd ? hi : lo;
+      const unsigned t0 = odd ? got : keep, t1 = odd ? keep : got;
+      const int d = 32 * dt + 8 * rg + 4 * h + (odd ? 2 : 0);
+      char* p = tile + d * TSTR + (w * QW + (r & ~1)) * 2;
+      *reinterpret_cast<unsigned*>(p) = (t0 & 0xffffu) | (t1 << 16);
+      *reinterpret_cast<unsigned*>(p + TSTR) = (t0 >> 16) | (t1 & 0xffff0000u);
+    }
+}
+
+template <int D>
+__device__ __forceinline__ void tile_store(const char* tile, unsigned short* dst, int64_t ld) {
+#pragma unroll
+  for (int i = 0; i < D / 16; ++i) {
+    const int c = threadIdx.x + i * NW * 64;
+    const int row = c >> 4, ch = c & 15;
+    *reinterpret_cast<u32x4*>(dst + (int64_t)row * ld + ch * 8) =
+        *reinterpret_cast<const u32x4*>(tile + row * TSTR + ch * 16);
+  }
+}
+
 template <bool MASK, int D, bool BAND = false>
 __device__ __forceinline__ void dq_tile(const LaneOffs<D>& lo, const char* kt, const char* vt, const bf16x8 (&qf)[D / 16],
                                         const bf16x8 (&df)[D / 16], f32x16 (&dqacc)[D / 32], float c, float lse2,
@@ -458,12 +531,13 @@
   }
 }
 
-template <bool SPARSE, int D, int NWF, bool BAND>
+template <bool SPARSE, int D, int NWF, bool BAND, bool EPI = false>
 __device__ __forceinline__ void dq_body(
     const unsigned short* __restrict__ q, Strides qs, const unsigned short* __restrict__ k, Strides ks,
     const unsigned short* __restrict__ v, Strides vs, const unsigned short* __restrict__ dout, Strides dos,
     const float* __restrict__ lse, const float* __restrict__ ndelta, unsigned short* __restrict__ dq, Strides dqs,
-    int B, int H, int Hk, int Sq, int Sk, float scale, int causal, Sparse sp, int kvlen, int qoff, Band bd) {
+    int B, int H, int Hk, int Sq, int Sk, float scale, int causal, Sparse sp, int kvlen, int qoff, Band bd,
+    const BwdEpi& ep = BwdEpi{}) {
   constexpr int ROWB = 2 * D;
   constexpr int BUF = 2 * KT * ROWB;
   int* tlist = reinterpret_cast<int*>(smem + 4 * KT * ROWB) + 1;
@@ -544,6 +618,31 @@
     if (t + 1 < ntiles) step(t + 1, std::integral_constant<int, 1>{});
   }
   unsigned short* op = dq + b * dqs.b + head * dqs.h + (int64_t)(q0 + r) * dqs.s;
+  if constexpr (EPI) {
+    static_assert(NWF == NW && D <= 128 && !SPARSE && kTileBytes<D> <= 2 * BUF, "EPI: 4 waves, head dims 64 / 128");
+#pragma unroll
+    for (int dt = 0; dt < D / 32; ++dt)
+#pragma unroll
+      for (int i = 0; i < 16; ++i) dqacc[dt][i] *= scale;
+    if (ep.rope.cos != nullptr && head < ep.rope.rot_heads_q)
+      rope_inv_acc<D>(dqacc, ep.rope, (int64_t)b * Sq + q0 + r, q0 + r, h);
+    u16x4 pk[D / 32][4];
+#pragma unroll
+    for (int dt = 0; dt < D / 32; ++dt)
+#pragma unroll
+      for (int rg = 0; rg < 4; ++rg) {
+#pragma unroll
+        for (int e = 0; e < 4; ++e) pk[dt][rg][e] = f32_to_bf16(dqacc[dt][4 * rg + e]);
+        *reinterpret_cast<u16x4*>(op + 32 * dt + 8 * rg + 4 * h) = pk[dt][rg];
+      }
+    if (ep.dt.q != nullptr) {
+      __syncthreads();
+      tile_put<D>(smem, pk, w, r, h);
+      __syncthreads();
+      tile_store<D>(smem, ep.dt.q + (int64_t)head * D * ep.dt.ld + (int64_t)b * Sq + qb * QBF, ep.dt.ld);
+    }
+    return;
+  }
 #pragma unroll
   for (int dt = 0; dt < D / 32; ++dt)
 #pragma unroll
@@ -563,6 +662,16 @@
     int B, int H, int Hk, int Sq, int Sk, float scale, int causal, Sparse sp, int kvlen, int qoff) {
   dq_body<SPARSE, D, NWF, false>(q, qs, k, ks, v, vs, dout, dos, lse, ndelta, dq, dqs, B, H, Hk, Sq, Sk, scale,
                                  causal, sp, kvlen, qoff, Band{nullptr, nullptr});
+}
+
+template <int D, bool BAND>
+__global__ void __launch_bounds__(NW * 64, (bwd_min_waves<D>())) dq_epi_kernel(
+    const unsigned short* __restrict__ q, Strides qs, const unsigned short* __restrict__ k, Strides ks,
+    const unsigned short* __restrict__ v, Strides vs, const unsigned short* __restrict__ dout, Strides dos,
+    const float* __restrict__ lse, const float* __restrict__ ndelta, unsigned short* __restrict__ dq, Strides dqs,
+    int B, int H, int Hk, int S, float scale, int causal, Band bd, BwdEpi ep) {
+  dq_body<false, D, NW, BAND, true>(q, qs, k, ks, v, vs, dout, dos, lse, ndelta, dq, dqs, B, H, Hk, S, S, scale,
+                                    BAND ? 1 : causal, Sparse{nullptr, 0, 0}, S, 0, bd, ep);
 }
 
 template <int D, int NWF = 4>
@@ -639,13 +748,14 @@
   }
 }
 
-template <bool SPLIT, int D, int PART, int NWK, bool BAND>
+template <bool SPLIT, int D, int PART, int NWK, bool BAND, bool EPI = false>
 __device__ __forceinline__ void dkdv_body(
     const unsigned short* __restrict__ q, Strides qs, const unsigned short* __restrict__ k, Strides ks,
     const unsigned short* __restrict__ v, Strides vs, const unsigned short* __restrict__ dout, Strides dos,
     const float* __restrict__ lse, const float* __restrict__ delta, unsigned short* __restrict__ dk, Strides dks,
     unsigned short* __restrict__ dv, Strides dvs, float* __restrict__ pk, float* __restrict__ pv, int B, int H,
-    int Hk, int Sq, int Sk, float scale, int causal, Sparse sp, int qoff, int hpw, Band bd) {
+    int Hk, int Sq, int Sk, float scale, int causal, Sparse sp, int qoff, int hpw, Band bd,
+    const BwdEpi& ep = BwdEpi{}) {
   constexpr int KB = NWK * QW;
   using G_ = KVL<D, KB>;
   char* vblk = smem;
@@ -749,6 +859,47 @@
   }
   unsigned short* kop = dk + b * dks.b + kh * dks.h + (int64_t)(k0 + r) * dks.s;
   unsigned short* vop = dv + b * dvs.b + kh * dvs.h + (int64_t)(k0 + r) * dvs.s;
+  if constexpr (EPI) {
+    static_assert(!SPLIT && NWK == NW && PART == 3 && D <= 128 && kTileBytes<D> <= G_::VBLK + 2 * G_::SLOT,
+                  "EPI: one sweep, 4 waves, head dims 64 / 128");
+#pragma unroll
+    for (int t = 0; t < D / 32; ++t)
+#pragma unroll
+      for (int i = 0; i < 16; ++i) dka[t][i] *= scale;
+    if (ep.rope.cos != nullptr && kh < ep.rope.rot_heads_k)
+      rope_inv_acc<D>(dka, ep.rope, (int64_t)b * Sk + k0 + r, k0 + r, h);
+    const int64_t tcol = (int64_t)kh * D * ep.dt.ld + (int64_t)b * Sk + kb * KB;
+    u16x4 pk4[D / 32][4];
+#pragma unroll
+    for (int t = 0; t < D / 32; ++t)
+#pragma unroll
+      for (int rg = 0; rg < 4; ++rg) {
+#pragma unroll
+        for (int e = 0; e < 4; ++e) pk4[t][rg][e] = f32_to_bf16(dka[t][4 * rg + e]);
+        *reinterpret_cast<u16x4*>(kop + 32 * t + 8 * rg + 4 * h) = pk4[t][rg];
+      }
+    if (ep.dt.q != nullptr) {
+      __syncthreads();
+      tile_put<D>(smem, pk4, w, r, h);
+      __syncthreads();
+      tile_store<D>(smem, ep.dt.k + tcol, ep.dt.ld);
+    }
+#pragma unroll
+    for (int t = 0; t < D / 32; ++t)
+#pragma unroll
+      for (int rg = 0; rg < 4; ++rg) {
+#pragma unroll
+        for (int e = 0; e < 4; ++e) pk4[t][rg][e] = f32_to_bf16(dva[t][4 * rg + e]);
+        *reinterpret_cast<u16x4*>(vop + 32 * t + 8 * rg + 4 * h) = pk4[t][rg];
+      }
+    if (ep.dt.q != nullptr) {
+      __syncthreads();
+      tile_put<D>(smem, pk4, w, r, h);
+      __syncthreads();
+      tile_store<D>(smem, ep.dt.v + tcol, ep.dt.ld);
+    }
+    return;
+  }
 #pragma unroll
   for (int t = 0; t < D / 32; ++t)
 #pragma unroll
@@ -775,6 +926,17 @@
                                         Hk, Sq, Sk, scale, causal, sp, qoff, hpw, Band{nullptr, nullptr});
 }
 
+template <int D, bool BAND>
+__global__ void __launch_bounds__(NW * 64, (bwd_min_waves<D>())) dkdv_epi_kernel(
+    const unsigned short* __restrict__ q, Strides qs, const unsigned short* __restrict__ k, Strides ks,
+    const unsigned short* __restrict__ v, Strides vs, const unsigned short* __restrict__ dout, Strides dos,
+    const float* __restrict__ lse, const float* __restrict__ delta, unsigned short* __restrict__ dk, Strides dks,
+    unsigned short* __restrict__ dv, Strides dvs, int B, int H, int Hk, int S, float scale, int causal, Band bd,
+    BwdEpi ep) {
+  dkdv_body<false, D, 3, NW, BAND, true>(q, qs, k, ks, v, vs, dout, dos, lse, delta, dk, dks, dv, dvs, nullptr, nullptr,
+                                         B, H, Hk, S, S, scale, BAND ? 1 : causal, Sparse{nullptr, 0, 0}, 0, 0, bd, ep);
+}
+
 template <bool SPLIT, int D, int PART = 3, int NWK = 4>
 __global__ void __launch_bounds__(NWK * 64, (NWK == 8 ? 1 : bwd_min_waves<D>())) dkdv_band_kernel(
     const unsigned short* __restrict__ q, Strides qs, const unsigned short* __restrict__ k, Strides ks,
@@ -787,16 +949,17 @@
 }
 
 
-template <int D>
+template <int D, bool ROPE = false>
 __global__ void __launch_bounds__(256) dkdv_reduce_kernel(const float* __restrict__ pk, const float* __restrict__ pv,
                                                           unsigned short* __restrict__ dk, Strides dks,
                                                           unsigned short* __restrict__ dv, Strides dvs, int B, int S,
-                                                          int H, int Hk) {
+                                                          int H, int Hk, RopeBwd rp = RopeBwd{}) {
   const int G = H / Hk;
-  const int64_t n8 = (int64_t)B * S * Hk * (D / 8);
+  constexpr int CPR = ROPE ? D / 16 : D / 8;
+  const int64_t n8 = (int64_t)B * S * Hk * CPR;
   for (int64_t i = (int64_t)blockIdx.x * blockDim.x + threadIdx.x; i < n8; i += (int64_t)gridDim.x * blockDim.x) {
-    const int c = (int)(i % (D / 8)) * 8;
-    const int64_t rest = i / (D / 8);
+    const int c = (int)(i % CPR) * 8;
+    const int64_t rest = i / CPR;
     const int kh = (int)(rest % Hk);
     const int64_t bs = rest / Hk;
     const int b = (int)(bs / S), s_ = (int)(bs - (int64_t)b * S);
@@ -809,8 +972,37 @@
 #pragma unroll
       for (int e = 0; e < 8; ++e) { ak[e] += x[e]; av[e] += y[e]; }
     }
-    store8<DT::BF16>(dk + b * dks.b + (int64_t)s_ * dks.s + kh * dks.h + c, ak);
-    store8<DT::BF16>(dv + b * dvs.b + (int64_t)s_ * dvs.s + kh * dvs.h + c, av);
+    unsigned short* kdst = dk + b * dks.b + (int64_t)s_ * dks.s + kh * dks.h + c;
+    unsigned short* vdst = dv + b * dvs.b + (int64_t)s_ * dvs.s + kh * dvs.h + c;
+    if constexpr (ROPE) {
+      constexpr int HALF = D / 2;
+      float bk[8] = {0, 0, 0, 0, 0, 0, 0, 0}, bv[8] = {0, 0, 0, 0, 0, 0, 0, 0};
+      for (int g = 0; g < G; ++g) {
+        const int64_t off = (bs * H + kh * G + g) * D + HALF + c;
+        float x[8], y[8];
+        load8<DT::F32>(pk + off, x);
+        load8<DT::F32>(pv + off, y);
+#pragma unroll
+        for (int e = 0; e < 8; ++e) { bk[e] += x[e]; bv[e] += y[e]; }
+      }
+      if (rp.cos != nullptr && kh < rp.rot_heads_k) {
+        int64_t p = rp.pos ? rp.pos[bs] : (int64_t)s_;
+        p = p < 0 ? 0 : (p >= rp.max_pos ? (int64_t)rp.max_pos - 1 : p);
+        float cs[8], sn[8];
+        load8<DT::F32>(rp.cos + p * HALF + c, cs);
+        load8<DT::F32>(rp.sin + p * HALF + c, sn);
+#pragma unroll
+        for (int e = 0; e < 8; ++e) {
+          const float a_ = ak[e], b_ = bk[e];
+          ak[e] = a_ * cs[e] + b_ * sn[e];
+          bk[e] = b_ * cs[e] - a_ * sn[e];
+        }
+      }
+      store8<DT::BF16>(kdst + HALF, bk);
+      store8<DT::BF16>(vdst + HALF, bv);
+    }
+    store8<DT::BF16>(kdst, ak);
+    store8<DT::BF16>(vdst, av);
   }
 }
 
@@ -945,10 +1137,11 @@
   return out;
 }
 
+constexpr int kEpiRope = 1, kEpiDualT = 2, kEpiDualTQ = 4;
 template <int D>
-static void bwd_impl_d(const at::Tensor& dout, const at::Tensor& q, const at::Tensor& k, const at::Tensor& v,
-                       const at::Tensor& o, const at::Tensor& lse, const at::Tensor& dq, const at::Tensor& dk,
-                       const at::Tensor& dv, double scale, const Mask& m) {
+static int bwd_impl_d(const at::Tensor& dout, const at::Tensor& q, const at::Tensor& k, const at::Tensor& v,
+                      const at::Tensor& o, const at::Tensor& lse, const at::Tensor& dq, const at::Tensor& dk,
+                      const at::Tensor& dv, double scale, const Mask& m, fa::BwdEpi ep = fa::BwdEpi{}) {
   using G_ = fa::KVL<D>;
   constexpr int KB8 = D == 128 ? 256 : fa::QB;
   static_assert(kRingBytes<D> + kListBytes <= kMaxDynamicLds, "dQ LDS exceeds the opt-in limit");
@@ -981,8 +1174,25 @@
   };
   const int dqw = env_int("SXE_FA_DQ_WAVES", 0);
   const bool dq8 = D < 256 && Sq % 256 == 0 && (dqw == 8 || (dqw == 0 && Sq >= 8192));
+  const int kvw = env_int("SXE_FA_DKDV_WAVES", 0);
+  const bool kv8 = D == 128 && Sk % 256 == 0 && (kvw == 8 || (kvw == 0 && Sk >= 8192));
+  const bool epi = D < 256 && (ep.rope.cos != nullptr || ep.dt.q != nullptr) && sp.layout == nullptr && !dq8 && !kv8 &&
+                   Sq == Sk && m.qoff == 0 && m.kvlen == Sk;
+  if (!epi) ep = fa::BwdEpi{};
+  int done = 0;
   if constexpr (D < 256) {
-    dq8 ? run_dq(int_t<8>{}) : run_dq(int_t<4>{});
+    if (epi) {
+      auto go = [&](auto kern) {
+        launch<decltype(kern)::value>((Sq / fa::QB) * B * H, fa::NW, kRingBytes<D>, u16(q), strides_of(q), u16(k),
+                                      strides_of(k), u16(v), strides_of(v), u16(dout), strides_of(dout),
+                                      lse.data_ptr<float>(), ndelta.data_ptr<float>(), u16(dq), strides_of(dq), B, H, Hk,
+                                      Sq, (float)scale, causal ? 1 : 0, m.bd, ep);
+      };
+      m.bd.klo != nullptr ? go(kern_t<fa::dq_epi_kernel<D, true>>{}) : go(kern_t<fa::dq_epi_kernel<D, false>>{});
+      done = (ep.rope.cos != nullptr ? kEpiRope : 0) | (ep.dt.q != nullptr ? kEpiDualTQ : 0);
+    } else {
+      dq8 ? run_dq(int_t<8>{}) : run_dq(int_t<4>{});
+    }
   } else {
     run_dq(int_t<4>{});
   }
@@ -1001,8 +1211,6 @@
   const bool partials = split && H / hpw > Hk;
   const int np = H / hpw;
   const bool one_sweep = D >= 256 && env_int("SXE_FA_DKDV_ONE_SWEEP", 1) != 0;
-  const int kvw = env_int("SXE_FA_DKDV_WAVES", 0);
-  const bool kv8 = D == 128 && Sk % 256 == 0 && (kvw == 8 || (kvw == 0 && Sk >= 8192));
   const size_t lds_kv = (kv8 ? fa::KVL<D, 256>::VBLK : G_::VBLK) + 2 * G_::SLOT + (sp.layout ? kListBytes : 0);
   at::Tensor pk, pv;
   if (partials) {
@@ -1042,20 +1250,43 @@
     run_dkdv(std::true_type{}, np);
     if (partials) {
       const int64_t n8 = (int64_t)B * Sk * Hk * (D / 8);
+      if constexpr (D < 256) {
+        if (ep.rope.cos != nullptr) {
+          hipLaunchKernelGGL((fa::dkdv_reduce_kernel<D, true>), dim3(stream_grid(n8 / 2, 256)), dim3(256), 0,
+                             cur_stream(), pk.data_ptr<float>(), pv.data_ptr<float>(), u16(dk), strides_of(dk), u16(dv),
+                             strides_of(dv), B, Sk, np, Hk, ep.rope);
+          SXE_LAUNCH_CHECK();
+          return done;
+        }
+      }
       hipLaunchKernelGGL(fa::dkdv_reduce_kernel<D>, dim3(stream_grid(n8, 256)), dim3(256), 0, cur_stream(),
                          pk.data_ptr<float>(), pv.data_ptr<float>(), u16(dk), strides_of(dk), u16(dv), strides_of(dv),
-                         B, Sk, np, Hk);
+                         B, Sk, np, Hk, fa::RopeBwd{});
       SXE_LAUNCH_CHECK();
     }
-  } else {
-    run_dkdv(std::false_type{}, Hk);
-  }
-}
-
-static void bwd_impl(at::Tensor dout, at::Tensor q, at::Tensor k, at::Tensor v, at::Tensor o, at::Tensor lse,
-                     at::Tensor dq, at::Tensor dk, at::Tensor dv, bool causal, double scale, fa::Sparse sp,
-                     int64_t kv_len = -1, int64_t causal_offset = INT64_MIN,
-                     fa::Band bd = kNoBand) {
+    return done;
+  }
+  if constexpr (D < 256) {
+    if (epi) {
+      auto go = [&](auto kern) {
+        launch<decltype(kern)::value>((Sk / fa::QB) * B * Hk, fa::NW, G_::VBLK + 2 * G_::SLOT, u16(q), strides_of(q),
+                                      u16(k), strides_of(k), u16(v), strides_of(v), u16(dout), strides_of(dout),
+                                      lse2.data_ptr<float>(), ndelta.data_ptr<float>(), u16(dk), strides_of(dk), u16(dv),
+                                      strides_of(dv), B, H, Hk, Sq, (float)scale, causal ? 1 : 0, m.bd, ep);
+      };
+      m.bd.klo != nullptr ? go(kern_t<fa::dkdv_epi_kernel<D, true>>{}) : go(kern_t<fa::dkdv_epi_kernel<D, false>>{});
+      if (ep.dt.q != nullptr) done = (done & ~kEpiDualTQ) | kEpiDualT;
+      return done;
+    }
+  }
+  run_dkdv(std::false_type{}, Hk);
+  return done;
+}
+
+static int bwd_impl(at::Tensor dout, at::Tensor q, at::Tensor k, at::Tensor v, at::Tensor o, at::Tensor lse,
+                    at::Tensor dq, at::Tensor dk, at::Tensor dv, bool causal, double scale, fa::Sparse sp,
+                    int64_t kv_len = -1, int64_t causal_offset = INT64_MIN,
+                    fa::Band bd = kNoBand, fa::BwdEpi ep = fa::BwdEpi{}) {
   check_qkv(q, k, v);
   check_qkv(dq, dk, dv);
   const Mask m = mask_of(q, k, causal, sp, kv_len, causal_offset, bd);
@@ -1064,9 +1295,11 @@
   SXE_CHECK(dq.sizes() == q.sizes() && dk.sizes() == k.sizes() && dv.sizes() == v.sizes(), "flash_attn_bwd: grad shapes");
   SXE_CHECK(lse.is_contiguous() && lse.size(2) == q.size(1), "flash_attn_bwd: lse [B, H, Sq]");
   c10::DeviceGuard guard(q.device());
+  int done = 0;
   dispatch_head_dim(q.size(3), "flash_attn_bwd", [&](auto d) {
-    bwd_impl_d<decltype(d)::value>(dout, q, k, v, o, lse, dq, dk, dv, scale, m);
+    done = bwd_impl_d<decltype(d)::value>(dout, q, k, v, o, lse, dq, dk, dv, scale, m, ep);
   });
+  return done;
 }
 
 static int64_t offset_arg(int64_t causal_offset) { return causal_offset == -(int64_t(1) << 40) ? INT64_MIN : causal_offset; }
@@ -1101,6 +1334,67 @@
 void flash_attn_bwd_band(at::Tensor dout, at::Tensor q, at::Tensor k, at::Tensor v, at::Tensor o, at::Tensor lse,
                          at::Tensor dq, at::Tensor dk, at::Tensor dv, at::Tensor klo, at::Tensor qhi, double scale) {
   bwd_impl(dout, q, k, v, o, lse, dq, dk, dv, true, scale, kNoSparse, -1, INT64_MIN, band_of(klo, qhi, q, k));
+}
+
+void rope_(at::Tensor x, at::Tensor cos_t, at::Tensor sin_t, c10::optional<at::Tensor> pos, int64_t seq_len,
+           int64_t pos_offset, bool inverse);
+void transpose16_into(const at::Tensor& x, const at::Tensor& y);
+
+void flash_attn_bwd_qkv(at::Tensor dout, at::Tensor q, at::Tensor k, at::Tensor v, at::Tensor o, at::Tensor lse,
+                        at::Tensor dq, at::Tensor dk, at::Tensor dv, c10::optional<at::Tensor> klo,
+                        c10::optional<at::Tensor> qhi, bool causal, double scale, c10::optional<at::Tensor> cos,
+                        c10::optional<at::Tensor> sin, c10::optional<at::Tensor> pos,
+                        c10::optional<at::Tensor> dqkvT) {
+  check_qkv(dq, dk, dv);
+  const int64_t B = dq.size(0), S = dq.size(1), Hq = dq.size(2), Hk = dk.size(2), D = dq.size(3);
+  const int64_t N = Hq + 2 * Hk, T = B * S;
+  SXE_CHECK(dk.size(1) == S && dq.stride(3) == 1 && dq.stride(2) == D && dq.stride(1) == N * D &&
+                dq.stride(0) == S * N * D && dk.strides() == dq.strides() && dv.strides() == dq.strides() &&
+                u16(dk) == u16(dq) + Hq * D && u16(dv) == u16(dk) + Hk * D,
+            "flash_attn_bwd_qkv: dq / dk / dv must be the head ranges of one contiguous [B, S, Hq + 2 Hkv, D] buffer");
+  const bool band = klo.has_value() && klo->defined();
+  SXE_CHECK(band == (qhi.has_value() && qhi->defined()), "flash_attn_bwd_qkv: klo and qhi come together");
+  const bool rope = cos.has_value() && cos->defined();
+  const bool has_pos = pos.has_value() && pos->defined();
+  fa::BwdEpi ep{};
+  if (rope) {
+    SXE_CHECK(sin.has_value() && sin->defined(), "flash_attn_bwd_qkv: cos and sin come together");
+    for (const at::Tensor* t : {&*cos, &*sin})
+      SXE_CHECK(t->is_cuda() && t->device() == dq.device() && t->scalar_type() == at::kFloat && t->is_contiguous() &&
+                    t->dim() == 2 && t->size(1) == D / 2 && t->size(0) >= 1 && t->size(0) == cos->size(0) &&
+                    (reinterpret_cast<uintptr_t>(t->data_ptr()) & 15) == 0,
+                "flash_attn_bwd_qkv: cos / sin must be contiguous fp32 [max_pos, D/2] on the device of dq");
+    if (has_pos) {
+      SXE_CHECK(pos->is_cuda() && pos->device() == dq.device() && pos->scalar_type() == at::kLong &&
+                    pos->is_contiguous() && pos->numel() == T,
+                "flash_attn_bwd_qkv: pos must be contiguous int64 [B * S] on the device of dq");
+    } else {
+      SXE_CHECK(S <= cos->size(0), "flash_attn_bwd_qkv: table too short for seq_len");
+    }
+    if (env_int("SXE_FA_BWD_ROPE", 1) != 0)
+      ep.rope = fa::RopeBwd{cos->data_ptr<float>(), sin->data_ptr<float>(), has_pos ? pos->data_ptr<int64_t>() : nullptr,
+                            (int)std::min<int64_t>(cos->size(0), INT32_MAX), (int)Hq, (int)Hk};
+  }
+  const bool dual = dqkvT.has_value() && dqkvT->defined();
+  if (dual) {
+    SXE_CHECK(dqkvT->is_cuda() && dqkvT->device() == dq.device() && dqkvT->scalar_type() == at::kBFloat16 &&
+                  dqkvT->is_contiguous() && dqkvT->dim() == 2 && dqkvT->size(0) == N * D && dqkvT->size(1) == T &&
+                  (reinterpret_cast<uintptr_t>(dqkvT->data_ptr()) & 15) == 0,
+              "flash_attn_bwd_qkv: dqkvT must be contiguous bf16 [(Hq + 2 Hkv) D, B S] on the device of dq");
+    if (env_int("SXE_FA_BWD_DUALT", 1) != 0) {
+      unsigned short* t0 = u16(*dqkvT);
+      ep.dt = fa::DualT{t0, t0 + Hq * D * T, t0 + (Hq + Hk) * D * T, T};
+    }
+  }
+  const int done = bwd_impl(dout, q, k, v, o, lse, dq, dk, dv, causal, scale, kNoSparse, -1, INT64_MIN,
+                            band ? band_of(*klo, *qhi, q, k) : kNoBand, ep);
+  if (rope && !(done & kEpiRope))
+    rope_(at::as_strided(dq, {B, S, Hq + Hk, D}, dq.strides()), *cos, *sin, pos, S, 0, true);
+  if (dual && !(done & kEpiDualT)) {
+    const int64_t c0 = (done & kEpiDualTQ) ? Hq * D : 0;
+    transpose16_into(at::as_strided(dq, {T, N * D - c0}, {N * D, 1}, dq.storage_offset() + c0),
+                     dqkvT->narrow(0, c0, N * D - c0));
+  }
 }
 
 template <int D>
@@ -1150,6 +1444,9 @@
   m.def("flash_attn_fwd_sparse(Tensor q, Tensor k, Tensor v, Tensor layout, int block, bool causal, float scale) -> Tensor[]");
   m.def("flash_attn_bwd_sparse(Tensor dout, Tensor q, Tensor k, Tensor v, Tensor o, Tensor lse, Tensor(a!) dq, "
         "Tensor(b!) dk, Tensor(c!) dv, Tensor layout, int block, bool causal, float scale) -> ()");
+  m.def("flash_attn_bwd_qkv(Tensor dout, Tensor q, Tensor k, Tensor v, Tensor o, Tensor lse, Tensor(a!) dq, "
+        "Tensor(b!) dk, Tensor(c!) dv, Tensor? klo, Tensor? qhi, bool causal, float scale, Tensor? cos, Tensor? sin, "
+        "Tensor? pos, Tensor(d!)? dqkvT) -> ()");
   m.def("flash_attn_fwd_band(Tensor q, Tensor k, Tensor v, Tensor klo, Tensor qhi, float scale) -> Tensor[]");
   m.def("flash_attn_bwd_band(Tensor dout, Tensor q, Tensor k, Tensor v, Tensor o, Tensor lse, Tensor(a!) dq, "
         "Tensor(b!) dk, Tensor(c!) dv, Tensor klo, Tensor qhi, float scale) -> ()");
@@ -1161,6 +1458,7 @@
   m.impl("flash_attn_bwd", &sxe::flash_attn_bwd);
   m.impl("flash_attn_fwd_sparse", &sxe::flash_attn_fwd_sparse);
   m.impl("flash_attn_bwd_sparse", &sxe::flash_attn_bwd_sparse);
+  m.impl("flash_attn_bwd_qkv", &sxe::flash_attn_bwd_qkv);
   m.impl("flash_attn_fwd_band", &sxe::flash_attn_fwd_band);
   m.impl("flash_attn_bwd_band", &sxe::flash_attn_bwd_band);
   m.impl("flash_attn_fwd_varlen", &sxe::flash_attn_fwd_varlen);
diff --git a/csrc/kernels/transpose.hip b/csrc/kernels/transpose.hip
--- a/csrc/kernels/transpose.hip
+++ b/csrc/kernels/transpose.hip
@@ -7,13 +7,14 @@
 constexpr int TLD = TT + 2;
 
 __global__ void __launch_bounds__(256) transpose16_kernel(const unsigned short* __restrict__ x,
-                                                          unsigned short* __restrict__ y, int64_t R, int64_t C) {
+                                                          unsigned short* __restrict__ y, int64_t R, int64_t C,
+                                                          int64_t ldx) {
   __shared__ unsigned short tile[TT * TLD];
   const int64_t tiles_c = C / TT;
   const int64_t tr = blockIdx.x / tiles_c, tc = blockIdx.x - tr * tiles_c;
   const int t = threadIdx.x;
   const int r = t >> 2, c0 = (t & 3) * 16;
-  const unsigned short* src = x + (tr * TT + r) * C + tc * TT + c0;
+  const unsigned short* src = x + (tr * TT + r) * ldx + tc * TT + c0;
   const u16x8 a = *reinterpret_cast<const u16x8*>(src);
   const u16x8 b = *reinterpret_cast<const u16x8*>(src + 8);
 #pragma unroll
@@ -34,21 +35,34 @@
   *reinterpret_cast<u16x8*>(dst + 8) = o1;
 }
 
+void transpose16_into(const at::Tensor& x, const at::Tensor& y) {
+  SXE_CHECK_CUDA(x);
+  SXE_CHECK(x.dim() == 2 && y.dim() == 2 && x.element_size() == 2 && y.scalar_type() == x.scalar_type() &&
+                y.device() == x.device(), "transpose16: 16-bit 2-D tensors of one dtype on one device");
+  const int64_t R = x.size(0), C = x.size(1), ldx = R > 1 ? x.stride(0) : C;
+  SXE_CHECK(y.is_contiguous() && y.size(0) == C && y.size(1) == R, "transpose16: output must be contiguous [C, R]");
+  SXE_CHECK((C <= 1 || x.stride(1) == 1) && ldx >= C && ldx % 8 == 0 &&
+                (reinterpret_cast<uintptr_t>(x.data_ptr()) & 15) == 0 && (reinterpret_cast<uintptr_t>(y.data_ptr()) & 15) == 0,
+            "transpose16: unit column stride and 16-byte aligned rows");
+  SXE_CHECK(R % TT == 0 && C % TT == 0, "transpose16: dims must be multiples of 64");
+  c10::DeviceGuard guard(x.device());
+  const int64_t tiles = (R / TT) * (C / TT);
+  if (tiles == 0) return;
+  SXE_CHECK(tiles < (1ll << 31), "transpose16: too many tiles");
+  hipLaunchKernelGGL(transpose16_kernel, dim3((unsigned)tiles), dim3(256), 0, cur_stream(),
+                     reinterpret_cast<const unsigned short*>(x.data_ptr()),
+                     reinterpret_cast<unsigned short*>(y.data_ptr()), R, C, ldx);
+  SXE_LAUNCH_CHECK();
+}
+
 at::Tensor transpose16(at::Tensor x) {
   SXE_CHECK_CUDA(x);
   SXE_CHECK(x.dim() == 2 && x.is_contiguous(), "transpose16: contiguous 2-D input");
   SXE_CHECK(x.element_size() == 2, "transpose16: 16-bit dtype");
   const int64_t R = x.size(0), C = x.size(1);
   SXE_CHECK(R % TT == 0 && C % TT == 0, "transpose16: dims must be multiples of 64");
-  c10::DeviceGuard guard(x.device());
   auto y = at::empty({C, R}, x.options());
-  const int64_t tiles = (R / TT) * (C / TT);
-  if (tiles == 0) return y;
-  SXE_CHECK(tiles < (1ll << 31), "transpose16: too many tiles");
-  hipLaunchKernelGGL(transpose16_kernel, dim3((unsigned)tiles), dim3(256), 0, cur_stream(),
-                     reinterpret_cast<const unsigned short*>(x.data_ptr()),
-                     reinterpret_cast<unsigned short*>(y.data_ptr()), R, C);
-  SXE_LAUNCH_CHECK();
+  transpose16_into(x, y);
   return y;
 }
 
diff --git a/shuffle_exchange_amd/ops/attention.py b/shuffle_exchange_amd/ops/attention.py
--- a/shuffle_exchange_amd/ops/attention.py
+++ b/shuffle_exchange_amd/ops/attention.py
@@ -128,6 +128,12 @@
         torch.ops.sxe.flash_attn_bwd(do, q, k, v, o, lse, dq, dk, dv, bool(causal), float(scale), *kv_args)
 
 
+def _flash_bwd_qkv(do, q, k, v, o, lse, dqkv, nq, nkv, causal, scale, klo, qhi, cos, sin, pos, dqkvT=None):
+    dq, dk, dv = dqkv[:, :, :nq], dqkv[:, :, nq:nq + nkv], dqkv[:, :, nq + nkv:]
+    torch.ops.sxe.flash_attn_bwd_qkv(do, q, k, v, o, lse, dq, dk, dv, klo, qhi, bool(causal), float(scale), cos, sin,
+                                     pos if cos is not None else None, dqkvT)
+
+
 def _pad_bounds(bounds, S_pad):
     klo, qhi = bounds
     B, S = klo.shape
@@ -226,12 +232,9 @@
     def backward(ctx, do):
         qkv, o, lse, cos, sin, pos, klo, qhi = ctx.saved_tensors
         nq, nkv, causal, scale = ctx.meta
-        dqkv = torch.empty_like(qkv)
+        dqkv = torch.empty_like(qkv, memory_format=torch.contiguous_format)
         q, k, v = qkv[:, :, :nq], qkv[:, :, nq:nq + nkv], qkv[:, :, nq + nkv:]
-        dq, dk, dv = dqkv[:, :, :nq], dqkv[:, :, nq:nq + nkv], dqkv[:, :, nq + nkv:]
-        _flash_bwd(do.contiguous(), q, k, v, o, lse, dq, dk, dv, causal, scale, klo, qhi)
-        if cos is not None:
-            torch.ops.sxe.rope_(dqkv[:, :, :nq + nkv], cos, sin, pos, qkv.shape[1], 0, True)
+        _flash_bwd_qkv(do.contiguous(), q, k, v, o, lse, dqkv, nq, nkv, causal, scale, klo, qhi, cos, sin, pos)
         return dqkv, None, None, None, None, None, None, None, None, None
 
 
@@ -282,18 +285,16 @@
         nq, nkv, causal, scale, x_shape = ctx.meta
         dqkv = torch.empty_like(qkv)
         q, k, v = qkv[:, :, :nq], qkv[:, :, nq:nq + nkv], qkv[:, :, nq + nkv:]
-        dq, dk, dv = dqkv[:, :, :nq], dqkv[:, :, nq:nq + nkv], dqkv[:, :, nq + nkv:]
-        _flash_bwd(do.contiguous(), q, k, v, o, lse, dq, dk, dv, causal, scale, klo, qhi)
+        d2 = dqkv.view(-1, w.shape[0])
+        d2T = d2.new_empty((d2.shape[1], d2.shape[0])) if ctx.needs_input_grad[1] else None
+        _flash_bwd_qkv(do.contiguous(), q, k, v, o, lse, dqkv, nq, nkv, causal, scale, klo, qhi, cos, sin, pos, d2T)
         del q, k, v, o, lse, qkv
-        if cos is not None:
-            torch.ops.sxe.rope_(dqkv[:, :, :nq + nkv], cos, sin, pos, dqkv.shape[1], 0, True)
-        d2 = dqkv.view(-1, w.shape[0])
         from .linear import data_grad
         from .mlp import weight_grad_tn
         dx = data_grad(d2, w).view(x_shape) if ctx.needs_input_grad[0] else None
         dw = None
         if ctx.needs_input_grad[1]:
-            dw = weight_grad_tn(w, torch.ops.sxe.transpose16(d2), xT, fp32_out=True)
+            dw = weight_grad_tn(w, d2T, xT, fp32_out=True)
         return dx, dw, None, None, None, None, None, None, None, None, None
 
 
diff --git a/shuffle_exchange_amd/ops/fake_kernels.py b/shuffle_exchange_amd/ops/fake_kernels.py
--- a/shuffle_exchange_amd/ops/fake_kernels.py
+++ b/shuffle_exchange_amd/ops/fake_kernels.py
@@ -86,6 +86,24 @@
     return None
 
 
+@_reg("sxe::flash_attn_bwd_qkv")
+def _fa_bwd_qkv(dout, q, k, v, o, lse, dq, dk, dv, klo, qhi, causal, scale, cos, sin, pos, dqkvT):
+    B, S, Hq, D = dq.shape
+    N = Hq + 2 * dk.shape[2]
+    torch._check(dq.shape == q.shape and dk.shape == k.shape and dv.shape == v.shape and dout.shape == q.shape,
+                 lambda: "flash_attn_bwd_qkv: grad shapes")
+    torch._check((cos is None) == (sin is None) and (klo is None) == (qhi is None),
+                 lambda: "flash_attn_bwd_qkv: cos / sin and klo / qhi come in pairs")
+    if cos is not None:
+        torch._check(cos.shape == sin.shape and cos.shape[-1] == D // 2, lambda: "flash_attn_bwd_qkv: cos / sin [max_pos, D/2]")
+    if pos is not None:
+        torch._check(pos.numel() == B * S, lambda: "flash_attn_bwd_qkv: pos [B * S]")
+    if dqkvT is not None:
+        torch._check(tuple(dqkvT.shape) == (N * D, B * S) and dqkvT.dtype == dq.dtype,
+                     lambda: f"flash_attn_bwd_qkv: dqkvT must be {(N * D, B * S)}, got {tuple(dqkvT.shape)}")
+    return None
+
+
 @_reg("sxe::flash_attn_fwd_varlen")
 def _fa_fwd_varlen(q, k, v, table, scale, window=0, out=None):
     return torch.empty_like(q, memory_format=torch.contiguous_format)
```

Result: no change. 26070 tokens/s, median of 6 (+0.2%).
